# Sun-Sir/BSARec

Hardware: AMD Instinct MI355X
Metric: train sequences/sec, ML-1M L=50 d=64 2-layer (higher is better)
Workload: dtype f32

## Files before the change

bsarec_amd/_lib.py:

```python
import ctypes as C
import os

HERE = os.path.dirname(os.path.abspath(__file__))
LIB_PATH = os.environ.get("BSAREC_LIB") or os.path.join(HERE, "libbsarec_hip.so")
MAX_LAYERS = 16
ABI_VERSION = 10
TOPK_MAX = 1024
NEG_MAX = 1024
NEG_MAX_DRAWS = 1 << 20
TRAIN_NEG_MAX = 8192
TRAIN_NEG_SITE = 0x4E454753

(BUF_LAYER_OUT, BUF_LOGITS, BUF_LOSS, BUF_DSP, BUF_HMIX, BUF_PROBS, BUF_DLAYER_IN, BUF_LOSS_ROWS, BUF_CTX,
 BUF_DLOGITS, BUF_TRAIN_CAND, BUF_TRAIN_CORR, BUF_TRAIN_LOGITS, BUF_TRAIN_DLOGITS) = range(14)
K_NONE, K_FFN1, K_FFN2, K_QKV, K_LOGITS, K_DU, K_DW1, K_FUSED_FWD, K_FUSED_BWD = range(9)

LAYER_FIELDS = ["sqrt_beta", "filter_ln_w", "filter_ln_b", "query_w", "query_b", "key_w", "key_b", "value_w", "value_b",
                "dense_w", "dense_b", "attn_ln_w", "attn_ln_b", "ffn1_w", "ffn1_b", "ffn2_w", "ffn2_b", "ffn_ln_w",
                "ffn_ln_b"]
LAYER_KEYS = {
    "sqrt_beta": "layer.filter_layer.sqrt_beta",
    "filter_ln_w": "layer.filter_layer.LayerNorm.weight", "filter_ln_b": "layer.filter_layer.LayerNorm.bias",
    "query_w": "layer.attention_layer.query.weight", "query_b": "layer.attention_layer.query.bias",
    "key_w": "layer.attention_layer.key.weight", "key_b": "layer.attention_layer.key.bias",
    "value_w": "layer.attention_layer.value.weight", "value_b": "layer.attention_layer.value.bias",
    "dense_w": "layer.attention_layer.dense.weight", "dense_b": "layer.attention_layer.dense.bias",
    "attn_ln_w": "layer.attention_layer.LayerNorm.weight", "attn_ln_b": "layer.attention_layer.LayerNorm.bias",
    "ffn1_w": "feed_forward.dense_1.weight", "ffn1_b": "feed_forward.dense_1.bias",
    "ffn2_w": "feed_forward.dense_2.weight", "ffn2_b": "feed_forward.dense_2.bias",
    "ffn_ln_w": "feed_forward.LayerNorm.weight", "ffn_ln_b": "feed_forward.LayerNorm.bias",
}
OPTIONAL_LAYER_KEYS = {"filter_cw": "layer.filter_layer.complex_weight"}
TOP_KEYS = {"item_emb": "item_embeddings.weight", "pos_emb": "position_embeddings.weight",
            "ln_w": "LayerNorm.weight", "ln_b": "LayerNorm.bias"}


class Config(C.Structure):
    _fields_ = [("batch", C.c_int), ("seq_len", C.c_int), ("hidden", C.c_int), ("heads", C.c_int), ("layers", C.c_int),
                ("item_size", C.c_int), ("cutoff_bins", C.c_int), ("alpha", C.c_float), ("ln_eps", C.c_float),
                ("p_hidden", C.c_float), ("p_attn", C.c_float), ("filter_kind", C.c_int),
                ("hidden_act", C.c_int), ("storage", C.c_int), ("no_fused", C.c_int), ("no_prune_top", C.c_int),
                ("dw_tiled", C.c_int), ("splits", C.c_int), ("top_slabs", C.c_int), ("separate_embed", C.c_int),
                ("separate_top", C.c_int), ("chain_kernels", C.c_int), ("x3_products", C.c_int),
                ("train_negatives", C.c_int), ("train_sampler", C.c_int), ("train_no_logq", C.c_int),
                ("train_lazy_adam", C.c_int)]


TRAIN_FIELDS = ("train_negatives", "train_sampler", "train_no_logq")
TRAIN_SAMPLERS = {"uniform": 0, "popularity": 1}


OPTION_FIELDS = ("storage", "no_fused", "no_prune_top", "dw_tiled", "splits", "top_slabs", "separate_embed", "separate_top", "chain_kernels", "x3_products")
HIDDEN_ACTS = {"gelu": 0, "relu": 1, "swish": 2, "tanh": 3, "sigmoid": 4}

_defaults = {k: 0 for k in OPTION_FIELDS}


def _env_defaults():
    e = os.environ
    d = {}
    if e.get("BSAREC_DW") == "tiled":
        d["dw_tiled"] = 1
    if e.get("BSAREC_PRUNE_TOP") == "0":
        d["no_prune_top"] = 1
    if e.get("BSAREC_EMBED_IN_BLOCK") == "0":
        d["separate_embed"] = 1
    if e.get("BSAREC_TOP_TAIL") == "0":
        d["separate_top"] = 1
    if e.get("BSAREC_FUSED") == "0":
        d["no_fused"] = 1
    if e.get("BSAREC_BLOCK_KERNELS") == "chain":
        d["chain_kernels"] = 1
    if e.get("BSAREC_PRODUCTS") == "bf16x3":
        d["x3_products"] = 1
    for env, key, hi in (("BSAREC_TOP_SLABS", "top_slabs", 16), ("BSAREC_SPLITS", "splits", 1024)):
        if e.get(env, "").isdigit() and 1 <= int(e[env]) <= hi:
            d[key] = int(e[env])
    if e.get("BSAREC_STORAGE") == "bf16":
        d["storage"] = 1
    return d


def set_default_options(**kw):
    old = {}
    for k, v in kw.items():
        if k not in _defaults:
            raise KeyError(k)
        old[k] = _defaults[k]
        _defaults[k] = int(v)
    return old


def default_options():
    d = dict(_defaults)
    d.update(_env_defaults())
    return d


class Layer(C.Structure):
    _fields_ = [(f, C.c_void_p) for f in LAYER_FIELDS] + [("filter_cw", C.c_void_p)]


class Tensors(C.Structure):
    _fields_ = [("item_emb", C.c_void_p), ("pos_emb", C.c_void_p), ("ln_w", C.c_void_p), ("ln_b", C.c_void_p),
                ("layer", Layer * MAX_LAYERS)]


class Adam(C.Structure):
    _fields_ = [("params", C.c_void_p), ("grads", C.c_void_p), ("exp_avg", C.c_void_p), ("exp_avg_sq", C.c_void_p),
                ("n", C.c_long), ("lr", C.c_float), ("beta1", C.c_float), ("beta2", C.c_float), ("eps", C.c_float),
                ("weight_decay", C.c_float), ("grad_scale", C.c_float), ("shadow_bf16", C.c_void_p), ("shadow_from", C.c_long),
                ("grads2", C.c_void_p), ("grads2_n", C.c_long), ("n_grad_srcs", C.c_int), ("grad_srcs", C.c_void_p * 8)]


class Comm(C.Structure):
    _fields_ = [("rank", C.c_int), ("world", C.c_int), ("flags", C.c_void_p * 8), ("epoch", C.c_void_p),
                ("error", C.c_void_p), ("timeout_ms", C.c_int)]


HOOK = C.CFUNCTYPE(None, C.c_void_p, C.c_void_p)


EXPORTS = {
    "bsarec_abi_version": (C.c_int, []),
    "bsarec_workspace_bytes": (C.c_size_t, [C.POINTER(Config)]),
    "bsarec_plan_create": (C.c_int, [C.POINTER(C.c_void_p), C.POINTER(Config), C.POINTER(Tensors), C.POINTER(Tensors),
                                     C.POINTER(Tensors), C.c_void_p, C.c_size_t, C.c_void_p, C.c_void_p, C.c_void_p]),
    "bsarec_shadow_refresh": (C.c_int, [C.c_void_p, C.c_void_p]),
    "bsarec_plan_set_dense_grad_hook": (C.c_int, [C.c_void_p, HOOK, C.c_void_p, C.c_void_p]),
    "bsarec_plan_set_train_sampler": (C.c_int, [C.c_void_p, C.c_void_p]),
    "bsarec_buffer_is_bf16": (C.c_int, [C.c_void_p, C.c_int, C.c_int]),
    "bsarec_plan_is_fused": (C.c_int, [C.c_void_p]),
    "bsarec_config_is_fused": (C.c_int, [C.c_void_p]),
    "bsarec_plan_destroy": (None, [C.c_void_p]),
    "bsarec_buffer_offset": (C.c_long, [C.c_void_p, C.c_int, C.c_int]),
    "bsarec_step_begin": (C.c_int, [C.c_void_p, C.c_void_p]),
    "bsarec_forward": (C.c_int, [C.c_void_p, C.c_void_p, C.c_int, C.c_void_p]),
    "bsarec_forward_last": (C.c_int, [C.c_void_p, C.c_void_p, C.c_int, C.c_void_p]),
    "bsarec_loss": (C.c_int, [C.c_void_p, C.c_void_p, C.c_void_p]),
    "bsarec_loss_bce": (C.c_int, [C.c_void_p, C.c_void_p, C.c_void_p, C.c_void_p]),
    "bsarec_loss_logsig": (C.c_int, [C.c_void_p, C.c_void_p, C.c_void_p, C.c_void_p]),
    "bsarec_logits": (C.c_int, [C.c_void_p, C.c_void_p]),
    "bsarec_backward": (C.c_int, [C.c_void_p, C.c_void_p]),
    "bsarec_backward_seq": (C.c_int, [C.c_void_p, C.c_void_p, C.c_void_p]),
    "bsarec_backward_seq_multi": (C.c_int, [C.c_void_p, C.c_void_p, C.c_void_p]),
    "bsarec_adam_step": (C.c_int, [C.POINTER(Adam), C.c_void_p, C.c_void_p]),
    "bsarec_train_step": (C.c_int, [C.c_void_p, C.c_void_p, C.c_void_p, C.POINTER(Adam), C.c_void_p]),
    "bsarec_gather_batch": (C.c_int, [C.c_void_p, C.c_void_p, C.c_void_p, C.c_long, C.c_void_p, C.c_int, C.c_int,
                                      C.c_void_p, C.c_void_p, C.c_void_p]),
    "bsarec_train_step_indexed": (C.c_int, [C.c_void_p] * 4 + [C.c_long] + [C.c_void_p] * 3 + [C.POINTER(Adam), C.c_void_p]),
    "bsarec_grad_step_indexed": (C.c_int, [C.c_void_p] * 4 + [C.c_long] + [C.c_void_p] * 3 + [C.c_float] * 3 + [C.c_void_p]),
    "bsarec_adam_apply": (C.c_int, [C.POINTER(Adam), C.c_void_p, C.c_void_p]),
    "bsarec_mask_seen": (C.c_int, [C.c_void_p, C.c_long, C.c_int, C.c_void_p, C.c_void_p, C.c_void_p, C.c_void_p]),
    "bsarec_topk_seen": (C.c_int, [C.c_void_p, C.c_long, C.c_int, C.c_int, C.c_void_p, C.c_void_p, C.c_void_p, C.c_int, C.c_void_p,
                                   C.c_void_p, C.c_void_p]),
    "bsarec_sampled_rank": (C.c_int, [C.c_void_p, C.c_long, C.c_void_p, C.c_int, C.c_int, C.c_int] + [C.c_void_p] * 5 +
                            [C.c_int, C.c_uint64, C.c_uint32] + [C.c_void_p] * 4),
    "bsarec_topk_full_workspace_bytes": (C.c_long, [C.c_int] * 5),
    "bsarec_topk_full": (C.c_int, [C.c_void_p, C.c_long, C.c_void_p, C.c_int, C.c_int, C.c_int] + [C.c_void_p] * 3 +
                         [C.c_int, C.c_int, C.c_void_p, C.c_long, C.c_void_p, C.c_void_p, C.c_void_p]),
    "bsarec_freq_layer_fwd": (C.c_int, [C.c_void_p] * 5 + [C.c_int] * 4 + [C.c_float, C.c_float, C.c_void_p, C.c_int,
# ... 91 lines not shown
```

bsarec_amd/csrc/bsarec_hip.hip:

```cpp
#include <cmath>
#include "../../include/bsarec_hip.h"
#include "../../include/bsarec_shard.h"
#include "epilogues.h"
#include "kernels.h"
#include "fused_layer.h"
#include "dw_direct.h"
#include "fused_top.h"
#include "fused_chain.h"
#include "comm.h"
#include "catalogue_shard.h"
#include "sampled_rank.h"
#include "full_rank.h"
#include "sampled_softmax.h"
#include "lazy_adam.h"

#include <hip/hip_runtime.h>
#include <math.h>
#include <stdio.h>
#include <stdlib.h>
#include <string.h>
#include <vector>
#include <algorithm>

#define HIPCHK(x) do { hipError_t e_ = (x); if (e_ != hipSuccess) return (int)e_; } while (0)
// ... 36 lines not shown
    float *xhat0, *rstd0;
    LayerBufs lb[BSAREC_MAX_LAYERS];
    float *logits, *dlogits, *loss_rows, *loss;
    float *dXa, *dXb, *dz, *dT, *dU, *dH, *dXacc, *dO, *dF, *dC, *dS, *dq, *dk, *dv, *dXtmp, *dlast_slab;
    float *slab_wL[BSAREC_MAX_LAYERS], *slab_bL[BSAREC_MAX_LAYERS], *part_lnL[BSAREC_MAX_LAYERS], *part_betaL[BSAREC_MAX_LAYERS];
    float *part_ln0, *part_pos, *trash;
    int pos_slices;
    ReduceJob* jobs; int jobs_per_layer;
    ReduceJob* jobs_pruned;
    bool prune_ok;
    bool pruned;
    int loss_kind;
    const float* ext_dy = nullptr;
    const float* ext_mid[BSAREC_MAX_LAYERS] = {};
    const int64_t *bce_pos, *bce_neg;
    float *part_kvb, *slab_dummy;
    float* part_cwL[BSAREC_MAX_LAYERS];
    float *top_dq, *top_dO, *top_dT, *top_dU, *top_ak, *top_rk, *top_av, *top_rv;
    int* blockmap; int red_blocks;
    long red_elems; const float *red_lo, *red_hi;
    int top_slabs; bool embed_in_block, direct_dw;
    bool scatter_in_block;
    ProfState prof;
    long long* stamps = nullptr;
    bsarec_hook_t dense_hook = nullptr; void* dense_hook_user = nullptr;
    float* lookup_grad = nullptr;
    unsigned long long* lookup_acc = nullptr;
    int* ssm_cand = nullptr; float *ssm_corr = nullptr, *ssm_logits = nullptr, *ssm_dlogits = nullptr;
    const int64_t* pop_cum = nullptr;
    const int64_t* ssm_answers = nullptr;
    int ssm_nslab = 0;
    LazyRows lazy = {};
    bool lazy_now = false;
};
struct PlanScope {
    bsarec_plan* prev;
    explicit PlanScope(bsarec_plan* p) : prev(t_plan) { t_plan = p; }
    ~PlanScope() { t_plan = prev; }
};

struct ProfScope {
    hipStream_t s; bool on; hipEvent_t stop;
    ProfScope(int kclass, hipStream_t st) : s(st), on(false) {
        ProfState* ps = t_plan ? &t_plan->prof : nullptr;
        on = ps && kclass != BSAREC_K_NONE && kclass == ps->kclass;
        if (!on) return;
        if (ps->used == ps->events.size()) {
            hipEvent_t a, b;
            (void)hipEventCreate(&a); (void)hipEventCreate(&b);
            ps->events.push_back({a, b});
        }
        (void)hipEventRecord(ps->events[ps->used].first, s);
        stop = ps->events[ps->used].second;
        ++ps->used;
    }
    ~ProfScope() { if (on) (void)hipEventRecord(stop, s); }
};

template <auto Kernel, class... A>
static int launch_lds(dim3 grid, dim3 block, size_t smem, hipStream_t s, const A&... a) {
    static size_t raised = 0;
    if (smem > 48 * 1024 && smem > raised) {
        HIPCHK(hipFuncSetAttribute(reinterpret_cast<const void*>(Kernel), hipFuncAttributeMaxDynamicSharedMemorySize, (int)smem));
        raised = smem;
    }
    if (g_dry) return 0;
// ... 41 lines not shown
    memset(&e, 0, sizeof(e));
    e.C[0] = C; e.ldc = ldc;
    return e;
}

struct Carver {
    char* base; size_t off;
    explicit Carver(char* b) : base(b), off(0) {}
    template <class T> T* take(size_t n) {
        T* p = base ? reinterpret_cast<T*>(base + off) : nullptr;
        off += rup((long)(n * sizeof(T)), 256);
        return p;
    }
};

static int check_cfg(const bsarec_config_t& c) {
    if (c.batch < 1 || c.seq_len < 1 || c.seq_len > 256) return -1;
    if (c.hidden < 4 || c.hidden > 256 || c.hidden % 4) return -2;
    if (c.heads < 1 || c.hidden % c.heads || (c.hidden / c.heads) % 4) return -3;
    if (c.layers < 1 || c.layers > BSAREC_MAX_LAYERS) return -4;
    if (c.item_size < 2) return -5;
    if (c.cutoff_bins < 1 || c.cutoff_bins > c.seq_len / 2 + 1) return -6;
    if ((long)c.cutoff_bins * c.hidden > 8192) return -7;
    if (c.p_hidden < 0.f || c.p_hidden >= 1.f || c.p_attn < 0.f || c.p_attn >= 1.f) return -8;
    if (c.filter_kind != 0 && c.filter_kind != 1) return -9;
    if (c.filter_kind == 1 && c.cutoff_bins != c.seq_len / 2 + 1) return -9;
    if (c.hidden_act < 0 || c.hidden_act > 4) return -14;
    if (c.storage < 0 || c.storage > 1) return -15;
    if (c.splits < 0 || c.splits > 1024 || c.top_slabs < 0 || c.top_slabs > 16) return -16;
    if (c.train_negatives < 0 || c.train_negatives > BSAREC_TRAIN_NEG_MAX) return -17;
    if (c.train_sampler < 0 || c.train_sampler > 1 || c.train_no_logq < 0 || c.train_no_logq > 1) return -17;
    if (c.train_negatives > 0 && c.storage != 0) return -18;
    if (c.train_lazy_adam < 0 || c.train_lazy_adam > 1 || (c.train_lazy_adam && c.train_negatives == 0)) return -19;
    return 0;
}

static bool fused_shape_ok(const bsarec_config_t& c) {
    const int dh = c.hidden / c.heads;
    if (c.no_fused || c.hidden_act != 0 || c.hidden != 64 || c.seq_len > 64 || !(dh == 16 || dh == 32 || dh == 64)) return false;
    if (c.filter_kind == 1) return c.storage == 0 && c.alpha == 1.0f && c.cutoff_bins <= 36;
    return c.cutoff_bins <= FUSED_MAX_CB;
}

#define SSM_SLAB_MAX 32
static void ssm_split(int N, int cap, int* nslab, int* chunk) {
    const int want = std::max(1, std::min(cap, N / 256));
    *chunk = (int)rup(cdiv(N, want), SSM_KS);
    *nslab = cdiv(N, *chunk);
}

static void derive(bsarec_plan& p) {
    const bsarec_config_t& c = p.cfg;
    p.fused = fused_shape_ok(c);
    p.bf = c.storage == 1 && p.fused;
    p.bf_products = c.storage == 1 && !p.fused;
    p.T = c.batch * c.seq_len;
    p.Lp = (int)rup(c.seq_len, 4);
    p.Vp = (int)rup(c.item_size, 4);
    p.dh = c.hidden / c.heads;
    p.nblk = p.fused ? c.batch : cdiv(p.T, 64);
    p.rows_pb = p.fused ? c.seq_len : 64;
    const int want_splits = c.splits > 0 ? c.splits : (p.fused ? 32 : 40);
    p.top_slabs = c.top_slabs > 0 ? c.top_slabs : 2;
    p.embed_in_block = !c.separate_embed || p.bf;
    p.direct_dw = !c.dw_tiled && (long)p.T * 4 * c.hidden * 4 < (1L << 31);
    p.scatter_in_block = p.fused && p.direct_dw && !c.separate_embed;
    long ch = rup(cdiv(p.T, want_splits), p.bf ? 2 * GEMM_BK : GEMM_BK);
// ... 69 lines not shown
}

extern "C" int bsarec_abi_version(void) { return BSAREC_ABI_VERSION; }

extern "C" size_t bsarec_workspace_bytes(const bsarec_config_t* cfg) {
    if (!cfg || check_cfg(*cfg) != 0) return 0;
    bsarec_plan p;
    p.cfg = *cfg;
    derive(p);
    size_t total = 0;
    carve(p, nullptr, &total);
    return total;
}

struct SlabMap { long wq, wk, wv, wo, w1, w2, wtot, bq, bk, bv, bo, b1, b2, btot; };
static SlabMap slab_map(long d) {
    SlabMap m;
    m.wq = 0; m.wk = d * d; m.wv = 2 * d * d; m.wo = 3 * d * d; m.w1 = 4 * d * d; m.w2 = 8 * d * d; m.wtot = 12 * d * d;
    m.bq = 0; m.bk = d; m.bv = 2 * d; m.bo = 3 * d; m.b1 = 4 * d; m.b2 = 8 * d; m.btot = 9 * d;
    return m;
}

static float* slab_w_ptr(const bsarec_plan& p, int l, long tensor_off) { return p.slab_wL[l] + tensor_off * p.nsplit; }
static float* slab_b_ptr(const bsarec_plan& p, int l, long tensor_off) { return p.slab_bL[l] + tensor_off * p.nsplit; }

enum LnPart { LN_FF_G, LN_FF_B, LN_A_G, LN_A_B, LN_F_G, LN_F_B };
enum Ln0Part { LN_E_G, LN_E_B };
static float* ln_part(const bsarec_plan& p, int l, LnPart k) { return p.part_lnL[l] + (long)k * p.nblk * p.cfg.hidden; }
static float* ln0_part(const bsarec_plan& p, Ln0Part k) { return p.part_ln0 + (long)k * p.nblk * p.cfg.hidden; }

static const float* h_last(const bsarec_plan& p) { return p.X[p.cfg.layers] + (long)(p.cfg.seq_len - 1) * p.cfg.hidden; }
static long h_last_stride(const bsarec_plan& p) { return (long)p.cfg.seq_len * p.cfg.hidden; }

extern "C" int bsarec_plan_create(bsarec_plan_t** out, const bsarec_config_t* cfg, const bsarec_tensors_t* params,
                                  const bsarec_tensors_t* grads, const bsarec_tensors_t* shadow, void* workspace,
                                  size_t workspace_bytes, void* state, const float* twiddle, void* stream) {
    if (!out || !cfg || !params || !workspace || !state || !twiddle) return -10;
    RET(check_cfg(*cfg));
    if (cfg->storage == 1 && fused_shape_ok(*cfg) && !shadow) return -15;
    if (((uintptr_t)workspace & 255) != 0) return -11;
    bsarec_plan* p = new bsarec_plan();
    p->cfg = *cfg;
    p->P = *params;
    if (grads) p->G = *grads; else memset(&p->G, 0, sizeof(p->G));
    if (shadow) p->S = *shadow; else memset(&p->S, 0, sizeof(p->S));
    p->ws = (char*)workspace; p->ws_bytes = workspace_bytes;
    p->state = (uint64_t*)state; p->twiddle = twiddle; p->train = false;
    derive(*p);
    size_t total = 0;
    carve(*p, p->ws, &total);
    if (total > workspace_bytes) { delete p; return -12; }
    if (hipMemset(p->lookup_acc, 0, (size_t)cfg->item_size * cfg->hidden * sizeof(unsigned long long)) != hipSuccess) {
        delete p; return -12;
    }
    if (cfg->train_lazy_adam && (hipMemset(p->lazy.mark, 0, (size_t)cfg->item_size * sizeof(int)) != hipSuccess ||
                                 hipMemset(p->lazy.count, 0, sizeof(int)) != hipSuccess)) {
        delete p; return -12;
    }

    const long d = cfg->hidden;
    const SlabMap sm = slab_map(d);
    std::vector<ReduceJob> jobs;
    auto add = [&](const float* src, float* dst, int nsplit, long len) {
        ReduceJob j; j.src = src; j.dst = dst; j.nsplit = nsplit; j.len = (int)len; j.stride = len; j.scale = 1.f; j.pad = 0;
        jobs.push_back(j);
    };
    const int ns = p->nsplit, nb = p->nblk;
    for (int l = 0; l < cfg->layers; ++l) {
        const bsarec_layer_t& g = p->G.layer[l];
        add(p->part_betaL[l], g.sqrt_beta, cfg->batch, d);
        add(ln_part(*p, l, LN_F_G), g.filter_ln_w, nb, d);
        add(ln_part(*p, l, LN_F_B), g.filter_ln_b, nb, d);
        add(slab_w_ptr(*p, l, sm.wq), g.query_w, ns, d * d); add(slab_b_ptr(*p, l, sm.bq), g.query_b, ns, d);
        add(slab_w_ptr(*p, l, sm.wk), g.key_w, ns, d * d);   add(slab_b_ptr(*p, l, sm.bk), g.key_b, ns, d);
        add(slab_w_ptr(*p, l, sm.wv), g.value_w, ns, d * d); add(slab_b_ptr(*p, l, sm.bv), g.value_b, ns, d);
        add(slab_w_ptr(*p, l, sm.wo), g.dense_w, ns, d * d); add(slab_b_ptr(*p, l, sm.bo), g.dense_b, ns, d);
        add(ln_part(*p, l, LN_A_G), g.attn_ln_w, nb, d);
        add(ln_part(*p, l, LN_A_B), g.attn_ln_b, nb, d);
        add(slab_w_ptr(*p, l, sm.w1), g.ffn1_w, ns, 4 * d * d); add(slab_b_ptr(*p, l, sm.b1), g.ffn1_b, ns, 4 * d);
        add(slab_w_ptr(*p, l, sm.w2), g.ffn2_w, ns, 4 * d * d); add(slab_b_ptr(*p, l, sm.b2), g.ffn2_b, ns, d);
        add(ln_part(*p, l, LN_FF_G), g.ffn_ln_w, nb, d);
        add(ln_part(*p, l, LN_FF_B), g.ffn_ln_b, nb, d);
    }
    add(ln0_part(*p, LN_E_G), p->G.ln_w, nb, d);
    add(ln0_part(*p, LN_E_B), p->G.ln_b, nb, d);
    if (p->scatter_in_block) {
        ReduceJob j; j.src = p->dz; j.dst = p->G.pos_emb; j.nsplit = cfg->batch; j.len = (int)((long)cfg->seq_len * d);
        j.stride = (long)cfg->seq_len * d; j.scale = 1.f; j.pad = 0;
        jobs.push_back(j);
    } else add(p->part_pos, p->G.pos_emb, p->pos_slices, (long)cfg->seq_len * d);
    if (cfg->filter_kind == 1)
        for (int l = 0; l < cfg->layers; ++l)
            add(p->part_cwL[l], p->G.layer[l].filter_cw, cfg->batch, (long)cfg->cutoff_bins * d * 2);
    p->jobs_per_layer = 19;
    p->prune_ok = p->fused && cfg->layers >= 2 && !cfg->no_prune_top && cfg->filter_kind == 0;
    p->pruned = false;
    p->loss_kind = 0; p->bce_pos = nullptr; p->bce_neg = nullptr;
    std::vector<ReduceJob> jobs_pr = jobs;
    {
        const size_t base = (size_t)(cfg->layers - 1) * 19;
        ReduceJob& jk = jobs_pr[base + 6]; jk.src = p->part_kvb; jk.nsplit = cfg->batch; jk.stride = d;
        ReduceJob& jv = jobs_pr[base + 8]; jv.src = p->part_kvb + (long)cfg->batch * d; jv.nsplit = cfg->batch; jv.stride = d;
        for (int j : {3, 4, 5, 7, 9, 10, 13, 14, 15, 16})
            jobs_pr[base + j].nsplit = std::min(p->top_slabs, ns);
    }
    std::vector<int> bmap;
    for (size_t j = 0; j < jobs.size(); ++j)
        for (int ch = 0; ch < cdiv(jobs[j].len, 64); ++ch) bmap.push_back((int)(j << 16) | ch);
    p->red_blocks = (int)bmap.size();
    p->red_elems = 0; p->red_lo = nullptr; p->red_hi = nullptr;
    for (const ReduceJob& j : jobs) {
        p->red_elems += j.len;
        if (!p->red_lo || j.dst < p->red_lo) p->red_lo = j.dst;
// ... 58 lines not shown
}

extern "C" int bsarec_plan_set_train_sampler(bsarec_plan_t* p, const int64_t* pop_cum) {
    if (!p) return -10;
    if (p->cfg.train_negatives == 0 || p->cfg.train_sampler != 1) return -22;
    p->pop_cum = pop_cum;
    return 0;
}

static int sampled_refusal(const bsarec_plan& p) {
    if (p.cfg.train_negatives == 0) return 0;
    if (p.dense_hook || p.lookup_grad) return -22;
    if (p.cfg.train_sampler == 1 && !p.pop_cum && !g_dry) return -23;
    return 0;
}

static int head_nsplit(const bsarec_plan& p) { return p.loss_kind == 1 ? 1 : (p.loss_kind == 2 ? p.ssm_nslab : p.vsplit); }

extern "C" int bsarec_plan_is_fused(const bsarec_plan_t* p) { return p && p->fused ? 1 : 0; }
extern "C" int bsarec_config_is_fused(const bsarec_config_t* cfg) {
    if (!cfg) return -10;
    RET(check_cfg(*cfg));
    return fused_shape_ok(*cfg) ? 1 : 0;
}

extern "C" int bsarec_buffer_is_bf16(const bsarec_plan_t* p, int buffer, int layer) {
    if (!p || !p->bf) return 0;
    switch (buffer) {
        case BSAREC_BUF_LAYER_OUT: return layer < p->cfg.layers ? 1 : 0;
        case BSAREC_BUF_HMIX: case BSAREC_BUF_PROBS: case BSAREC_BUF_CTX: return 1;
        case BSAREC_BUF_DLAYER_IN: return 1;
        default: return 0;
    }
}

extern "C" int bsarec_shadow_refresh(bsarec_plan_t* p, void* stream) {
    if (!p) return -10;
    if (!p->bf) return 0;
    const long d = p->cfg.hidden;
    for (int l = 0; l < p->cfg.layers; ++l) {
        const bsarec_layer_t& w = p->P.layer[l];
        const bsarec_layer_t& sh = p->S.layer[l];
        CastJobs6 J;
        const float* src[6] = {w.query_w, w.key_w, w.value_w, w.dense_w, w.ffn1_w, w.ffn2_w};
        float* dst[6] = {sh.query_w, sh.key_w, sh.value_w, sh.dense_w, sh.ffn1_w, sh.ffn2_w};
        for (int i = 0; i < 6; ++i) { J.src[i] = src[i]; J.dst[i] = (unsigned short*)dst[i]; J.n4[i] = (i < 4 ? d * d : 4 * d * d) / 4; }
        hipLaunchKernelGGL(cast_bf16_kernel, dim3(cdiv(4 * d * d / 4, ROW_THREADS), 6), dim3(ROW_THREADS), 0, (hipStream_t)stream, J);
        HIPCHK(hipGetLastError());
    }
    return 0;
}

static uint32_t drop_thresh(float p) {
    double t = (double)p * 4294967296.0;
    if (t <= 0) return 0;
    if (t >= 4294967295.0) return 0xFFFFFFFFu;
    return (uint32_t)t;
}
static DropP make_drop(const bsarec_plan& p, float prob, int site, bool train) {
    DropP d;
    d.thresh = train ? drop_thresh(prob) : 0;
    d.scale = (train && prob > 0.f) ? (float)(1.0 / (1.0 - (double)prob)) : 1.0f;
    d.rng = p.state; d.site = (uint32_t)site;
    return d;
}
static int lpr_for(int d) { return d <= 64 ? 16 : (d <= 128 ? 32 : 64); }
// ... 63 lines not shown
    F.xhat_f = b.xhat_f; F.rstd_f = b.rstd_f; F.q = b.q; F.k = b.k; F.v = b.v; F.probs = b.probs;
    F.xhat_a = b.xhat_a; F.rstd_a = b.rstd_a; F.xhat_ff = b.xhat_ff; F.rstd_ff = b.rstd_ff;
    F.L = c.seq_len; F.Lp = p.Lp; F.cb = c.cutoff_bins; F.heads = c.heads;
    F.alpha = c.alpha; F.oma = (float)(1.0 - (double)c.alpha);
    F.drop_f = make_drop(p, c.p_hidden, 1 + 4 * l, tr); F.drop_p = make_drop(p, c.p_attn, 2 + 4 * l, tr);
    F.drop_o = make_drop(p, c.p_hidden, 3 + 4 * l, tr); F.drop_ff = make_drop(p, c.p_hidden, 4 + 4 * l, tr);
    F.stamps = p.stamps ? p.stamps + 32 * (2 * l + (FWD ? 0 : 1)) : nullptr;
    if constexpr (FWD) {
        F.Xout = p.X[l + 1];
        F.f_b = w.filter_ln_b; F.bq = w.query_b; F.bk = w.key_b; F.bv = w.value_b; F.bo = w.dense_b; F.a_b = w.attn_ln_b;
        F.b1 = w.ffn1_b; F.b2 = w.ffn2_b; F.ff_b = w.ffn_ln_b;
        F.ids32 = p.ids32; F.ctx = b.ctx; F.hmix = b.hmix; F.u = b.u;
        F.eps = c.ln_eps;
    }
}

template <class BlockP>
static void fill_block_partials(const bsarec_plan& p, int l, BlockP& F) {
    F.pg_ff = ln_part(p, l, LN_FF_G); F.pb_ff = ln_part(p, l, LN_FF_B); F.pg_a = ln_part(p, l, LN_A_G);
    F.pb_a = ln_part(p, l, LN_A_B); F.pg_f = ln_part(p, l, LN_F_G); F.pb_f = ln_part(p, l, LN_F_B);
    F.pbeta = p.part_betaL[l];
}

static void fill_top_fwd(bsarec_plan& p, int l, bool tr, TopFwdP& F) {
    fill_block<true>(p, l, tr, p.P.layer[l], F);
    F.low = p.lb[l].dsp;
    F.wk_sh = p.S.layer[l].key_w; F.wv_sh = p.S.layer[l].value_w;
}

static int launch_fused_fwd(bsarec_plan& p, int l, bool tr, hipStream_t s, const int64_t* ids = nullptr, const GatherP* gp = nullptr,
                            bool top_tail = false ) {
    const bsarec_config_t& c = p.cfg;
    FusedFwdP F;
    fill_block<true>(p, l, tr, p.bf ? p.S.layer[l] : p.P.layer[l], F);
    F.xout_f32 = (l == c.layers - 1);
    F.gp = p.lb[l].gp;
    F.dsp = nullptr;
    if (l == 0 && gp) {
        F.e_E = p.P.item_emb; F.e_pos = p.P.pos_emb; F.e_g = p.P.ln_w; F.e_b = p.P.ln_b; F.e_ids = ids; F.e_gp = *gp;
        F.e_drop = make_drop(p, c.p_hidden, 0, tr); F.e_V = c.item_size;
        F.e_X0 = p.X[0]; F.e_xhat = p.xhat0; F.e_rstd = p.rstd0; F.e_ids32 = p.ids32;
    }
    F.trash = p.trash;
    TopFwdP TF;
    if (top_tail) fill_top_fwd(p, l + 1, tr, TF);
    const dim3 grid(c.batch), block(512);
    ProfScope prof(BSAREC_K_FUSED_FWD, s);
    if (c.filter_kind == 1) {
        F.filter_cw = p.P.layer[l].filter_cw;
        return launch_lds<fused_layer_fwd_kernel<32, false, NoTail, false, true>>(grid, block, fused_fwd_smem_bytes(), s, F, NoTail());
    }
    int rc = 0;
    if (!p.bf && c.chain_kernels && !c.x3_products) {
        const size_t csm = fused_chain_fwd_smem_bytes(top_tail);
        DISPATCH_DH(p.dh, rc = top_tail ? launch_lds<fused_chain_fwd_kernel<DH, TopFwdP>>(grid, block, csm, s, F, TF)
                                        : launch_lds<fused_chain_fwd_kernel<DH, NoTail>>(grid, block, csm, s, F, NoTail()));
        return rc;
    }
    const size_t smem = fused_fwd_smem_bytes();
    DISPATCH_BLOCK(p, rc = top_tail ? launch_lds<fused_layer_fwd_kernel<DH, BF, TopFwdP, X3>>(grid, block, smem, s, F, TF)
                                    : launch_lds<fused_layer_fwd_kernel<DH, BF, NoTail, X3>>(grid, block, smem, s, F, NoTail()));
    return rc;
}

static int launch_fused_bwd(bsarec_plan& p, int l, bool tr, const float* dY, float* dXout, hipStream_t s, bool top,
                            const TopBwdP* head = nullptr ) {
    const bsarec_config_t& c = p.cfg;
    FusedBwdP F;
    fill_block<false>(p, l, tr, p.bf ? p.S.layer[l] : p.P.layer[l], F);
    fill_block_partials(p, l, F);
    F.dY = dY; F.dX = dXout;
    F.u = p.lb[l].gp;
    if (top) { F.dh_slabs = p.dlast_slab; F.dh_nsplit = head_nsplit(p); F.dh_stride = (long)c.batch * c.hidden; }
    if (l == 0) {
        F.e_dz = p.dz; F.e_xhat = p.xhat0; F.e_rstd = p.rstd0; F.e_g = p.P.ln_w;
        F.e_pg = ln0_part(p, LN_E_G); F.e_pb = ln0_part(p, LN_E_B); F.e_drop = make_drop(p, c.p_hidden, 0, tr);
        F.e_dx_extra = p.ext_dy ? p.ext_mid[0] : nullptr;
    }
    F.dT = p.dT; F.dU = p.dU; F.dO = p.dO; F.dq = p.dq; F.dk = p.dk; F.dv = p.dv;
    F.trash = p.trash;
    const dim3 grid(c.batch), block(512);
    const size_t smem = fused_bwd_smem_bytes();
    ProfScope prof(BSAREC_K_FUSED_BWD, s);
    if (c.filter_kind == 1) {
        F.filter_cw = p.P.layer[l].filter_cw; F.pcw = p.part_cwL[l];
        return launch_lds<fused_layer_bwd_kernel<32, false, NoTail, false, true>>(grid, block, smem, s, F, NoTail());
    }
    int rc = 0;
    DISPATCH_BLOCK(p, rc = head ? launch_lds<fused_layer_bwd_kernel<DH, BF, TopBwdP, X3>>(grid, block, smem, s, F, *head)
                                : launch_lds<fused_layer_bwd_kernel<DH, BF, NoTail, X3>>(grid, block, smem, s, F, NoTail()));
    return rc;
}

static int launch_top_fwd(bsarec_plan& p, int l, bool tr, hipStream_t s) {
    TopFwdP F;
    fill_top_fwd(p, l, tr, F);
    int rc = 0;
    DISPATCH_BLOCK(p, rc = launch_lds<top_fwd_kernel<DH, BF>>(dim3(p.cfg.batch), dim3(256), top_fwd_smem_bytes(), s, F));
    return rc;
}

static void fill_top_bwd(bsarec_plan& p, int l, bool tr, float* dXout, TopBwdP& F) {
    const bsarec_config_t& c = p.cfg;
    fill_block<false>(p, l, tr, p.P.layer[l], F);
    fill_block_partials(p, l, F);
    F.dX = dXout;
    F.u = p.lb[l].u; F.low = p.lb[l].dsp;
    F.dh_slabs = p.dlast_slab; F.dh_nsplit = head_nsplit(p); F.dh_stride = (long)c.batch * c.hidden;
    F.dT = p.top_dT; F.dU = p.top_dU; F.dO = p.top_dO; F.dq = p.top_dq;
    F.ak = p.top_ak; F.rk = p.top_rk; F.av = p.top_av; F.rv = p.top_rv;
    F.pbk = p.part_kvb; F.pbv = p.part_kvb + (long)c.batch * c.hidden;
}

static int launch_top_bwd(bsarec_plan& p, int l, bool tr, float* dXout, hipStream_t s) {
    TopBwdP F;
    fill_top_bwd(p, l, tr, dXout, F);
    int rc = 0;
    DISPATCH_BLOCK(p, rc = launch_lds<top_bwd_kernel<DH, BF>>(dim3(p.cfg.batch), dim3(256), top_bwd_smem_bytes(), s, F));
    return rc;
}

// ... 534 lines not shown
}

static int launch_dw_grouped(const bsarec_plan& p, const GroupedTN& G, hipStream_t s) {
    ProfScope prof(BSAREC_K_DW1, s);
    const dim3 grid(G.tile0[6], p.nsplit), block(GEMM_THREADS);
    if (!p.bf_products)
        return launch_lds<gemm_grouped_tn_kernel<false, 64>>(grid, block, GemmSmem<64, 64, true, true, false>::BYTES, s, G);
    if (dw_tile(p) == 128)
        return launch_lds<gemm_grouped_tn_kernel<true, 128>>(grid, block, GemmSmem<128, 128, true, true, true>::BYTES, s, G);
    return launch_lds<gemm_grouped_tn_kernel<true, 64>>(grid, block, GemmSmem<64, 64, true, true, true>::BYTES, s, G);
}

static int embed_bwd(bsarec_plan& p, const float* dY, hipStream_t s) {
    const bsarec_config_t& c = p.cfg;
    const int T = p.T, d = c.hidden, L = c.seq_len, B = c.batch;
    if (!p.fused) {
        LnBranch a; memset(&a, 0, sizeof(a));
        a.xhat = p.xhat0; a.rstd = p.rstd0; a.gamma = p.P.ln_w; a.in_scale = 1.f;
        a.drop = make_drop(p, c.p_hidden, 0, p.train); a.dT = nullptr;
        a.pgamma = ln0_part(p, LN_E_G); a.pbeta = ln0_part(p, LN_E_B);
        DISPATCH_LPR(d, LAUNCH((ln_bwd_kernel<LPR, 2>), dim3(p.nblk), dim3(ROW_THREADS), 0, s, dY, a, a, p.dz, T, d, p.rows_pb));
        HIPCHK(hipGetLastError());
    }
    if (!p.scatter_in_block)
    DISPATCH_LPR(d, {
        constexpr int CHUNK = SCATTER_FLOATS / (LPR * 4);
        const int sb = cdiv(T, CHUNK);
        RET(launch_lds<embed_bwd_kernel<LPR>>(dim3(sb + L * p.pos_slices), dim3(ROW_THREADS), SCATTER_FLOATS * 8 + 2 * CHUNK * 4, s,
                                              p.dz, p.ids32, B, L, d, p.lookup_acc, p.part_pos, sb));
    });
    return 0;
}

static int final_reduce(bsarec_plan& p, const TickP& tick, const bsarec_adam_t* fuse_adam, hipStream_t s) {
    const bsarec_config_t& c = p.cfg;
    LookupAcc la;
    memset(&la, 0, sizeof(la));
    la.acc = p.lookup_acc; la.dst = p.lookup_grad ? p.lookup_grad : p.G.item_emb; la.n4 = (long)c.item_size * c.hidden / 4;
    la.nblocks = (int)std::min<long>(cdiv(la.n4, ROW_THREADS), 1024);
    la.dense_zero = (!p.ext_dy && p.loss_kind == 2) ? 1 : 0;
    const bool lazy = p.lazy_now && !p.ext_dy && p.loss_kind == 2;
    if (lazy) {
        la.lazy = p.lazy;
        la.nblocks = (int)std::min<long>(cdiv((long)p.lazy.cap * p.lazy.d4, ROW_THREADS), 1024);
    }
    const ReduceJob* jobs = p.pruned ? p.jobs_pruned : p.jobs;
    if (fuse_adam) {
        const bsarec_adam_t& a = *fuse_adam;
        AdamFuseP A;
        memset(&A, 0, sizeof(A));
        A.w = a.params; A.g = const_cast<float*>(a.grads); A.m = a.exp_avg; A.v = a.exp_avg_sq;
        A.b1 = a.beta1; A.b2 = a.beta2; A.eps = a.eps; A.wd = a.weight_decay;
        A.shadow = (unsigned short*)a.shadow_bf16; A.shadow_from = a.shadow_bf16 ? a.shadow_from : a.n;
        A.item_off = p.G.item_emb - a.grads; A.item_n4 = la.n4; A.lookup_acc = la.acc;
        A.dense_zero = la.dense_zero;
        if (lazy) A.lazy = p.lazy;
        int ab = lazy ? la.nblocks : cdiv(A.item_n4, ROW_THREADS);
        if (ab > 1024) ab = 1024;
        LAUNCH(reduce_adam_kernel, dim3(p.red_blocks + ab), dim3(ROW_THREADS), 0, s, jobs, p.blockmap, p.red_blocks,
               (const uint64_t*)p.state, A);
    } else
        LAUNCH(multi_reduce_flat_kernel, dim3(p.red_blocks + la.nblocks + (tick.state ? 1 : 0)), dim3(ROW_THREADS), 0, s, jobs,
               p.blockmap, p.red_blocks, tick, la);
    return (int)hipGetLastError();
}

static int backward_impl(bsarec_plan_t* p, void* stream, const TickP& tick, const bsarec_adam_t* fuse_adam) {
    if (!p) return -10;
    if (!p->G.item_emb) return -13;
    if (fuse_adam && p->lookup_grad) return -21;
    PlanScope scope(p);
    hipStream_t s = (hipStream_t)stream;
    const bsarec_config_t& c = p->cfg;
    const int T = p->T, d = c.hidden, L = c.seq_len, B = c.batch, N = c.layers;
    const bool tr = p->train;

    RET(head_bwd(*p, s));
    if (p->dense_hook && !g_dry && !p->ext_dy) p->dense_hook(p->dense_hook_user, stream);
    float* dY = (N & 1) ? p->dXb : p->dXa;
    RET(top_grad(*p, dY, s));

    DwPending pend;
    memset(&pend, 0, sizeof(pend));
    for (int l = N - 1; l >= 0; --l) {
        float* dXout = (dY == p->dXa) ? p->dXb : p->dXa;
        const bool top_pruned = p->fused && p->pruned && l == N - 1;
        if (top_pruned) {
            if (N >= 2 && !c.separate_top && p->direct_dw) { fill_top_bwd(*p, l, tr, dXout, pend.top_head); pend.have_head = true; }
// ... 25 lines not shown
}

static TickP make_tick(void* state, int adam, float lr, float b1, float b2, const float* loss_rows, int B, float* loss_out,
                       void* cursor, int advance, int bump_step) {
    TickP t;
    memset(&t, 0, sizeof(t));
    t.state = (uint64_t*)state; t.adam = adam; t.lr = lr; t.b1 = b1; t.b2 = b2;
    t.loss_rows = loss_rows; t.B = B; t.loss_out = loss_out;
    t.cursor = (long long*)cursor; t.advance = advance; t.bump_step = bump_step;
    return t;
}

static int adam_check(const bsarec_adam_t* a) {
    if (!a || !a->params || !a->grads || !a->exp_avg || !a->exp_avg_sq || a->n <= 0 || (a->n & 3)) return -10;
    if (a->shadow_bf16 && (a->shadow_from < 0 || (a->shadow_from & 3))) return -10;
    if (a->grads2 && (a->grads2_n < 0 || a->grads2_n > a->n || (a->grads2_n & 3))) return -10;
    if (a->n_grad_srcs < 0 || a->n_grad_srcs > 8) return -10;
    for (int r = 0; r < a->n_grad_srcs; ++r) if (!a->grad_srcs[r]) return -10;
    return 0;
}

static int adam_launch(const bsarec_adam_t& a, void* state, hipStream_t s) {
    const long n4 = a.n / 4;
    int blocks = cdiv(n4, ROW_THREADS);
    if (blocks > 2048) blocks = 2048;
    GradSrcs S;
    memset(&S, 0, sizeof(S));
    S.nsrc = a.n_grad_srcs;
    for (int r = 0; r < a.n_grad_srcs; ++r) S.src[r] = a.grad_srcs[r];
    S.g2 = a.grads2; S.n2_4 = a.grads2 ? a.grads2_n / 4 : 0;
    LAUNCH(adam_kernel, dim3(blocks), dim3(ROW_THREADS), 0, s, a.params, a.grads, a.exp_avg, a.exp_avg_sq, n4,
           (const uint64_t*)state, a.beta1, a.beta2, a.eps, a.weight_decay, a.grad_scale, (unsigned short*)a.shadow_bf16,
           a.shadow_bf16 ? a.shadow_from / 4 : n4, S);
    return (int)hipGetLastError();
}

extern "C" int bsarec_adam_step(const bsarec_adam_t* a, void* state, void* stream) {
    RET(adam_check(a));
    if (!state) return -10;
    hipStream_t s = (hipStream_t)stream;
    LAUNCH(adam_tick_kernel, dim3(1), dim3(ROW_THREADS), 0, s, make_tick(state, 1, a->lr, a->beta1, a->beta2, nullptr, 0, nullptr, nullptr, 0, 0));
    HIPCHK(hipGetLastError());
    return adam_launch(*a, state, s);
}

extern "C" int bsarec_adam_apply(const bsarec_adam_t* a, void* state, void* stream) {
    RET(adam_check(a));
    if (!state) return -10;
    return adam_launch(*a, state, (hipStream_t)stream);
}

static int lazy_check(const bsarec_plan& p, const bsarec_adam_t& a) {
    if (!p.cfg.train_lazy_adam) return 0;
    if (a.grads2 || a.n_grad_srcs > 0 || a.shadow_bf16) return -24;
    const long item = (long)p.cfg.item_size * p.cfg.hidden;
    if (!p.G.item_emb || p.G.item_emb < a.grads) return -24;
    const long off = p.G.item_emb - a.grads;
    if (off + item > a.n || (off & 3)) return -24;
    return 0;
}

static int lazy_adam_launch(const bsarec_plan& p, const bsarec_adam_t& a, hipStream_t s) {
    LazyAdamP A;
    memset(&A, 0, sizeof(A));
    A.w = a.params; A.g = a.grads; A.m = a.exp_avg; A.v = a.exp_avg_sq;
    A.n = a.n; A.item_off = p.G.item_emb - a.grads; A.item_n = (long)p.cfg.item_size * p.cfg.hidden;
    A.b1 = a.beta1; A.b2 = a.beta2; A.eps = a.eps; A.wd = a.weight_decay; A.gscale = a.grad_scale;
// ... 5 lines not shown
}

struct LazyStep {
    bsarec_plan* p;
    explicit LazyStep(bsarec_plan* q) : p(q) { p->lazy_now = p->cfg.train_lazy_adam != 0; }
    ~LazyStep() { p->lazy_now = false; }
};

extern "C" int bsarec_gather_batch(const int64_t* table, const int64_t* answers_table, const int64_t* perm, long n_samples,
                                   const void* cursor, int B, int L, int64_t* ids_out, int64_t* answers_out, void* stream) {
    if (!table || !answers_table || !perm || !cursor || !ids_out || !answers_out || B < 1 || L < 1) return -10;
    LAUNCH(gather_batch_kernel, dim3(cdiv((long)B * L, ROW_THREADS)), dim3(ROW_THREADS), 0, (hipStream_t)stream, table,
           answers_table, perm, n_samples, (const long long*)cursor, B, L, ids_out, answers_out);
    return (int)hipGetLastError();
}

extern "C" int bsarec_train_step_indexed(bsarec_plan_t* p, const int64_t* table, const int64_t* answers_table,
                                         const int64_t* perm, long n_samples, void* cursor, int64_t* ids_buf,
                                         int64_t* answers_buf, const bsarec_adam_t* a, void* stream) {
    if (!p) return -10;
    RET(adam_check(a));
    RET(sampled_refusal(*p));
    RET(lazy_check(*p, *a));
    hipStream_t s = (hipStream_t)stream;
    if (!table || !answers_table || !perm || !cursor || !ids_buf || !answers_buf) return -10;
    LazyStep lazy(p);
    GatherP gp{table, answers_table, perm, n_samples, (const long long*)cursor, ids_buf, answers_buf};
    RET(forward_impl(p, ids_buf, 1, stream, gp, true));
    RET(loss_impl(p, answers_buf, stream, false));
    const TickP tk = make_tick(p->state, 1, a->lr, a->beta1, a->beta2, p->loss_rows, p->cfg.batch, p->loss, cursor, p->cfg.batch, 1);
    if (can_fuse_adam(*p, *a) && !p->cfg.separate_embed)
        return backward_impl(p, stream, tk, a);
    RET(backward_impl(p, stream, tk));
    return p->lazy_now ? lazy_adam_launch(*p, *a, s) : adam_launch(*a, p->state, s);
}

extern "C" int bsarec_grad_step_indexed(bsarec_plan_t* p, const int64_t* table, const int64_t* answers_table,
                                        const int64_t* perm, long n_samples, void* cursor, int64_t* ids_buf,
                                        int64_t* answers_buf, float lr, float b1, float b2, void* stream) {
    if (!p || !table || !answers_table || !perm || !cursor || !ids_buf || !answers_buf) return -10;
    RET(sampled_refusal(*p));
    if (p->cfg.train_lazy_adam) return -22;
    GatherP gp{table, answers_table, perm, n_samples, (const long long*)cursor, ids_buf, answers_buf};
    RET(forward_impl(p, ids_buf, 1, stream, gp, true));
    RET(bsarec_loss(p, answers_buf, stream));
    return backward_impl(p, stream, make_tick(p->state, lr > 0.f ? 1 : 0, lr, b1, b2, nullptr, 0, nullptr, cursor, p->cfg.batch, 1));
}

extern "C" int bsarec_train_step(bsarec_plan_t* p, const int64_t* ids, const int64_t* answers, const bsarec_adam_t* a,
                                 void* stream) {
    if (!p) return -10;
    RET(adam_check(a));
    RET(sampled_refusal(*p));
    RET(lazy_check(*p, *a));
    if (p->cfg.train_lazy_adam) {
        LazyStep lazy(p);
        RET(bsarec_step_begin(p, stream));
        RET(bsarec_forward_last(p, ids, 1, stream));
        RET(bsarec_loss(p, answers, stream));
        TickP tk = make_tick(p->state, 1, a->lr, a->beta1, a->beta2, nullptr, 0, nullptr, nullptr, 0, 0);
        RET(backward_impl(p, stream, tk));
        return lazy_adam_launch(*p, *a, (hipStream_t)stream);
    }
    RET(bsarec_step_begin(p, stream));
    RET(bsarec_forward_last(p, ids, 1, stream));
    RET(bsarec_loss(p, answers, stream));
    RET(bsarec_backward(p, stream));
    return bsarec_adam_step(a, p->state, stream);
}

extern "C" int bsarec_mask_seen(float* scores, long ld, int B, const int64_t* users, const int64_t* indptr,
                                const int64_t* indices, void* stream) {
    if (!scores || !users || !indptr || !indices || B < 1 || ld < 1) return -10;
    hipLaunchKernelGGL(mask_seen_kernel, dim3(B), dim3(ROW_THREADS), 0, (hipStream_t)stream, scores, ld, users, indptr, indices);
    return (int)hipGetLastError();
}

extern "C" int bsarec_topk_seen(float* scores, long ld, int B, int V, const int64_t* users, const int64_t* indptr,
                                const int64_t* indices, int k, int64_t* out_idx, float* out_val, void* stream) {
    static_assert(BSAREC_TOPK_MAX == TOPK_MAX && ROW_THREADS == 256, "topk_seen_kernel: one thread per digit bin");
    if (!scores || !out_idx || B < 1 || V < 1 || ld < V || k < 1 || k > BSAREC_TOPK_MAX || k > V) return -10;
    if (indptr && (!users || !indices)) return -10;
    hipLaunchKernelGGL(topk_seen_kernel, dim3(B), dim3(ROW_THREADS), 0, (hipStream_t)stream, scores, ld, V, users, indptr, indices, k,
                       out_idx, out_val);
    return (int)hipGetLastError();
}

extern "C" int bsarec_sampled_rank(const float* h, long ldh, const float* item_emb, int B, int V, int d, const int64_t* users,
                                   const int64_t* answers, const int64_t* indptr, const int64_t* indices, const int64_t* pop_cum,
                                   int n_neg, uint64_t seed, uint32_t tag, int32_t* rank_out, int64_t* cand_out, float* score_out,
                                   void* stream) {
    static_assert(BSAREC_NEG_MAX == NEG_MAX && BSAREC_NEG_MAX_DRAWS == NEG_MAX_DRAWS, "sampled_rank_kernel: the header's limits");
    if (!h || !item_emb || !users || !answers || !rank_out || (indptr && !indices)) return -10;
    if (B < 1 || V < 2 || d < 4 || d > 256 || d % 4 != 0 || ldh < d || n_neg < 1 || n_neg > BSAREC_NEG_MAX) return -10;
    if ((uintptr_t)item_emb % 16 != 0) return -10;
    hipLaunchKernelGGL(sampled_rank_kernel, dim3(B), dim3(ROW_THREADS), 0, (hipStream_t)stream, h, ldh, item_emb, V, d, users, answers,
                       indptr, indices, pop_cum, n_neg, (uint32_t)seed, (uint32_t)(seed >> 32), tag, rank_out, cand_out, score_out);
    return (int)hipGetLastError();
}

struct FrShape { long s, stride, cap; };
// ... 364 lines not shown
```

bsarec_amd/csrc/fused_layer.h:

```cpp
#pragma once
#include "common.h"
#include "kernels.h"
#include <type_traits>

#define FS 68
#define FU 260
#define FUSED_MAX_CB 8

struct FusedFwdP {
    const float* X; float* Xout;
    const float *sqrt_beta, *f_g, *f_b, *wq, *bq, *wk, *bk, *wv, *bv, *wo, *bo, *a_g, *a_b, *w1, *b1, *w2, *b2, *ff_g, *ff_b;
    const float* tw; const int* ids32;
    float *xhat_f, *rstd_f, *q, *k, *v, *probs, *ctx, *xhat_a, *rstd_a, *hmix, *u, *xhat_ff, *rstd_ff, *dsp;
    float* gp;
    int L, Lp, cb, heads;
    float alpha, oma, eps;
    DropP drop_f, drop_p, drop_o, drop_ff;
    float* trash;
    long long* stamps;
    const float *e_E, *e_pos, *e_g, *e_b; const int64_t* e_ids; GatherP e_gp; DropP e_drop; int e_V;
    float *e_X0, *e_xhat, *e_rstd; int* e_ids32;
    int xout_f32;
    const float* filter_cw;
};


template <class T> struct GlobalPtr { static __device__ __forceinline__ T fix(T v) { return v; } };
template <class U> struct GlobalPtr<U*> {
    static __device__ __forceinline__ U* fix(U* v) {
        return (U*)(__attribute__((address_space(1))) U*)v;
    }
};
template <class T>
__device__ __forceinline__ T kernarg_field(unsigned byte_off) {
    typedef __attribute__((address_space(4))) const char* kptr_t;
// ... 121 lines not shown
        const float c = tab[2 * (k * 64 + t)] * w, sn = tab[2 * (k * 64 + t) + 1] * w;
        low += ld4(spec + (k * 2 + 0) * 64 + lc) * c - ld4(spec + (k * 2 + 1) * 64 + lc) * sn;
    }
    return low * (1.0f / (float)L);
}

template <int MM, int K> struct WFrag;
template <int K> struct WFrag<0, K> { f32x4 w[K / 8]; };
template <int K> struct WFrag<1, K> { u32x4 w[K / 16]; };
template <int K> struct WFrag<2, K> { f32x4 w[K / 8]; };

struct Split3 { u32x4 h, m, l; };
__device__ __forceinline__ f32x4 bf_lo4(const u32x4& p, int half) {
    return half == 0 ? f32x4{bf_lo(p.x), bf_hi(p.x), bf_lo(p.y), bf_hi(p.y)} : f32x4{bf_lo(p.z), bf_hi(p.z), bf_lo(p.w), bf_hi(p.w)};
}
__device__ __forceinline__ Split3 split3(f32x4 a0, f32x4 a1) {
    Split3 r;
    r.h = pk8(a0, a1);
    a0 = a0 - bf_lo4(r.h, 0); a1 = a1 - bf_lo4(r.h, 1);
    r.m = pk8(a0, a1);
    a0 = a0 - bf_lo4(r.m, 0); a1 = a1 - bf_lo4(r.m, 1);
    r.l = pk8(a0, a1);
    return r;
}
__device__ __forceinline__ f32x16 mfma_x3(const Split3& a, const Split3& b, f32x16 acc) {
    acc = mfma_bf16(a.l, b.h, acc);
    acc = mfma_bf16(a.h, b.l, acc);
    acc = mfma_bf16(a.m, b.m, acc);
    acc = mfma_bf16(a.m, b.h, acc);
    acc = mfma_bf16(a.h, b.m, acc);
    return mfma_bf16(a.h, b.h, acc);
}

template <int MM, int K>
__device__ __forceinline__ void load_w(const float* __restrict__ base, long e, WFrag<MM, K>& f) {
    if constexpr (MM == 1) {
#pragma unroll
        for (int s = 0; s < K / 16; ++s) f.w[s] = *reinterpret_cast<const AS_GLOBAL u32x4*>((const AS_GLOBAL char*)base + 2 * (e + 16 * s));
    } else if constexpr (MM == 2) {
#pragma unroll
        for (int s = 0; s < K / 16; ++s) { f.w[2 * s] = gld4(base + e + 16 * s); f.w[2 * s + 1] = gld4(base + e + 16 * s + 4); }
    } else {
#pragma unroll
        for (int kb = 0; kb < K / 8; ++kb) f.w[kb] = gld4(base + e + 8 * kb);
    }
}
template <int MM, int K, int LDW>
__device__ __forceinline__ void load_wT(const float* __restrict__ base, long e, WFrag<MM, K>& f) {
    if constexpr (MM == 1) {
        const AS_GLOBAL unsigned short* g = reinterpret_cast<const AS_GLOBAL unsigned short*>((const AS_GLOBAL char*)base + 2 * e);
#pragma unroll
        for (int s = 0; s < K / 16; ++s) {
            unsigned h[8];
#pragma unroll
            for (int j = 0; j < 8; ++j) h[j] = g[(16 * s + j) * LDW];
            f.w[s] = u32x4{h[0] | (h[1] << 16), h[2] | (h[3] << 16), h[4] | (h[5] << 16), h[6] | (h[7] << 16)};
        }
    } else if constexpr (MM == 2) {
        const float* gw = base + e;
#pragma unroll
        for (int s = 0; s < K / 16; ++s) {
            f.w[2 * s] = f32x4{gld(gw + (16 * s + 0) * LDW), gld(gw + (16 * s + 1) * LDW), gld(gw + (16 * s + 2) * LDW), gld(gw + (16 * s + 3) * LDW)};
            f.w[2 * s + 1] = f32x4{gld(gw + (16 * s + 4) * LDW), gld(gw + (16 * s + 5) * LDW), gld(gw + (16 * s + 6) * LDW), gld(gw + (16 * s + 7) * LDW)};
        }
    } else {
        const float* gw = base + e;
#pragma unroll
        for (int kb = 0; kb < K / 8; ++kb) {
            f.w[kb].x = gld(gw + (8 * kb + 0) * LDW); f.w[kb].y = gld(gw + (8 * kb + 1) * LDW);
            f.w[kb].z = gld(gw + (8 * kb + 2) * LDW); f.w[kb].w = gld(gw + (8 * kb + 3) * LDW);
        }
    }
}
template <int MM, int K>
__device__ __forceinline__ void mma_w(const float* __restrict__ sa, const WFrag<MM, K>& f, f32x16& acc) {
    if constexpr (MM == 1) {
#pragma unroll
        for (int s = 0; s < K / 16; ++s) acc = mfma_bf16(pk8(ld4(sa + 16 * s), ld4(sa + 16 * s + 4)), f.w[s], acc);
    } else if constexpr (MM == 2) {
#pragma unroll
        for (int s = 0; s < K / 16; ++s)
            acc = mfma_x3(split3(ld4(sa + 16 * s), ld4(sa + 16 * s + 4)), split3(f.w[2 * s], f.w[2 * s + 1]), acc);
// ... 50 lines not shown
        const bool ok = r < L;
        const long e = (tok0 + r) * 64 + lc;
        f32x4 v = {0, 0, 0, 0};
        if (ok) v = (ld4(tileA + r * FS + lc) + ld4(tileB + r * FS + lc) + P.bi) * P.dm[i] + ld4(resid + r * FS + lc);
        const float mean = group_sum<16>(v.x + v.y + v.z + v.w) * (1.0f / 64.0f);
        f32x4 dl = {0, 0, 0, 0};
        if (ok) dl = v - mean;
        const float var = group_sum<16>(dl.x * dl.x + dl.y * dl.y + dl.z * dl.z + dl.w * dl.w) * (1.0f / 64.0f);
        const float rs = 1.0f / sqrtf(var + eps);
        f32x4 y = {0, 0, 0, 0};
        if (ok) {
            const f32x4 xh = dl * rs;
            y = P.g * xh + P.be;
            if (MIX) y = alpha * ld4(dsp + r * FS + lc) + oma * y;
            ast4<BF>(xhatG, e, xh);
            if (BF && out_f32) gst4(outG + e, y); else ast4<BF>(outG, e, y);
            if (lc == 0) gst(rstdG + tok0 + r, rs);
        }
        if (BF && round_outL) {
            const unsigned a = pk_bf16(y.x, y.y), c = pk_bf16(y.z, y.w);
            y = f32x4{bf_lo(a), bf_hi(a), bf_lo(c), bf_hi(c)};
        }
        if (outL) st4(outL + r * FS + lc, y);
    }
}

struct NoTail {};
template <bool BF> struct TopFwdRegs;
template <bool BF, unsigned KOFF, bool KV> __device__ __forceinline__ void top_fwd_prefetch(TopFwdRegs<BF>& R);
template <int DH, bool BF, unsigned KOFF, bool HELPED>
__device__ __forceinline__ void top_fwd_rest(const TopFwdRegs<BF>& R, const DropSeed& dseed, float* sX, float* sK, float* sV,
                                             float* sPart, float* sTab, float* sSpec, float* sVec, const int* sIds);
template <bool BF> struct TopFwdHelpRegs;
template <bool BF, unsigned KOFF> __device__ __forceinline__ void top_fwd_help_prefetch(TopFwdHelpRegs<BF>& H);
template <int DH, bool BF, unsigned KOFF>
__device__ __forceinline__ void top_fwd_help(const TopFwdHelpRegs<BF>& H, const float* sX, float* sK, float* sV, float* sVec);
template <class T> struct IsTail { static constexpr bool value = true; };
template <> struct IsTail<NoTail> { static constexpr bool value = false; };
constexpr int TOP_BWD_BARRIERS = 11;
struct TopBwdRegs {
    float sl[32];
    float xh_ff, g_ff, rs_ff, xa, xf, g_a, g_f, rs_a, rs_f, bt, low_l, x_l, q_l;
    f32x4 tq[16];
    float p_pre;
};
struct TopBwdHelpRegs { f32x4 w2c[16], w1c[16], u4; };
template <bool BF, unsigned KOFF> __device__ __forceinline__ void top_bwd_prefetch(TopBwdRegs& R);
template <bool BF, unsigned KOFF> __device__ __forceinline__ void top_bwd_prefetch_tile(TopBwdRegs& R);
template <bool BF, unsigned KOFF> __device__ __forceinline__ void top_bwd_help_prefetch(TopBwdHelpRegs& H);
template <int DH, bool BF, unsigned KOFF, bool HELPED>
__device__ __forceinline__ void top_bwd_body(const TopBwdRegs& R, const DropSeed& dseed, float* sX, float* sK, float* sV, const float* sTab,
                                             float* sVec, float* sDX);
template <bool BF, unsigned KOFF> __device__ __forceinline__ void top_bwd_help_a(const TopBwdHelpRegs& H, float* sVec);
template <int DH, bool BF, unsigned KOFF> __device__ __forceinline__ void top_bwd_help_b(const float* sX, float* sVec, const float* gu, f32x4 (&uw)[16]);


template <int DH, bool BF, class TAILP, bool X3 = false, bool FM = false>
__global__ void __launch_bounds__(512) __attribute__((amdgpu_waves_per_eu(2, 2)))
fused_layer_fwd_kernel(const FusedFwdP P_unused, const TAILP T_unused) {
#define PTYPE FusedFwdP
    static_assert(!(BF && X3), "x3 products work on fp32 tensors");
    constexpr int MM = X3 ? 2 : (BF ? 1 : 0);
    static_assert(!FM || (!BF && !X3 && !IsTail<TAILP>::value), "the FMLPRec block runs in fp32, without a top-block tail");
    constexpr int MAXCB = FM ? 36 : FUSED_MAX_CB;
    constexpr bool TAIL = IsTail<TAILP>::value;
    constexpr unsigned KOFF = (unsigned)((sizeof(FusedFwdP) + 7) & ~(size_t)7);
    const auto R0_L = KARG(FusedFwdP, L);
    const auto R0_Lp = KARG(FusedFwdP, Lp);
    const auto R0_cb = KARG(FusedFwdP, cb);
    const auto R0_heads = KARG(FusedFwdP, heads);
    extern __shared__ __attribute__((aligned(16))) float sm[];
    constexpr int TS = 64 * FS;
    float* sX = sm;
    float* sD = sm + TS;
    float* sH = sm + 2 * TS;
    float* sE = sm + 3 * TS;
    float* sR = sm + 4 * TS;
    float* sQ = sR;
    float* sK = sR + TS;
    float* sVt = sR + 2 * TS;
    float* sC = sR + 3 * TS;
    float* sU = sR;
    float* sTab = sR + 4 * TS;
    float* sSpec = sTab + FUSED_MAX_CB * 128;
    float* sRed = sSpec + FUSED_MAX_CB * 128;
    int* sIds = reinterpret_cast<int*>(sRed + 512);
    if constexpr (FM) { sTab = sR; sSpec = sR + 2 * TS; }

    const int tid = threadIdx.x, lane = tid & 63, wave = tid >> 6;
    const int l31 = lane & 31, half = lane >> 5;
    const int grp = wave >> 2, wm = (wave >> 1) & 1, wn = wave & 1;
    const int L = R0_L, Lp = R0_Lp, heads = R0_heads, cb = R0_cb;
    const int b = blockIdx.x;
    const long tok0 = (long)b * L;
    const int col = wn * 32 + l31;
    constexpr int KHM = MM ? 8 : 4;
    const int KH = KHM * half;
    const long wrow = (long)col * 64 + KH;
    const int arow = (wm * 32 + l31) * FS + KH;
    float* const trash = KARG(FusedFwdP, trash) + 4 * lane;

    STAMP(0);
    const KernargTouch ktouch = kernarg_touch<IsTail<TAILP>::value ? KOFF + (unsigned)sizeof(TAILP) : (unsigned)sizeof(FusedFwdP)>();
    const DropSeed dseed = drop_seed(KARG(FusedFwdP, drop_f));
    kernarg_touch_done(ktouch);
    const auto R1_X = KARG(FusedFwdP, X);
    const auto R1_ids32 = KARG(FusedFwdP, ids32);
    const auto R1_tw = KARG(FusedFwdP, tw);
    const auto R1_wq = KARG(FusedFwdP, wq);
    WFrag<MM, 64> wA, wB;
    float qkv_bias[3] = {0.f, 0.f, 0.f};
    if (!FM && grp == 1) {
        load_w<MM, 64>(R1_wq, wrow, wA);
        qkv_bias[0] = gld(KARG(FusedFwdP, bq) + col); qkv_bias[1] = gld(KARG(FusedFwdP, bk) + col);
        qkv_bias[2] = gld(KARG(FusedFwdP, bv) + col);
    }
    const float* const eE = KARG(FusedFwdP, e_E);
    if (eE) {
        const GatherP gp = KARG(FusedFwdP, e_gp);
        const int64_t* const eids = KARG(FusedFwdP, e_ids);
        const float* const epos = KARG(FusedFwdP, e_pos);
        const int V = KARG(FusedFwdP, e_V);
        const float eeps = KARG(FusedFwdP, eps);
        const float* const e_g = KARG(FusedFwdP, e_g); const float* const e_b = KARG(FusedFwdP, e_b);
        int* const e_ids32 = KARG(FusedFwdP, e_ids32); const DropP e_drop = KARG(FusedFwdP, e_drop);
        float* const e_xhat = KARG(FusedFwdP, e_xhat); float* const e_X0 = KARG(FusedFwdP, e_X0); float* const e_rstd = KARG(FusedFwdP, e_rstd);
        long src = 0;
        if (gp.table) {
            src = *(const AS_GLOBAL long long*)gp.cursor + b;
            src = src < gp.n ? (long)*(const AS_GLOBAL int64_t*)(gp.perm + src) : 0;
            if (tid == 0) *(AS_GLOBAL int64_t*)(gp.ans_out + b) = *(const AS_GLOBAL int64_t*)(gp.ans_table + src);
        }
        const f32x4 eg = gld4(e_g + ((tid & 15) << 2)), eb = gld4(e_b + ((tid & 15) << 2));
#pragma unroll
        for (int p = 0; p < 2; ++p) {
            const int idx = tid + p * 512, r = idx >> 4, c4 = (idx & 15) << 2;
            const bool ok = r < L;
            const long e = (tok0 + r) * 64 + c4;
            f32x4 v = {0, 0, 0, 0};
            int id = 0;
            if (ok) {
                int64_t id64;
                if (gp.table) {
                    id64 = *(const AS_GLOBAL int64_t*)(gp.table + src * L + r);
                    if (c4 == 0) *(AS_GLOBAL int64_t*)(gp.ids_out + tok0 + r) = id64;
                } else id64 = *(const AS_GLOBAL int64_t*)(eids + tok0 + r);
// ... 26 lines not shown
        st4(sX + r * FS + c4, v);
    }
    if (tid < 64) sIds[tid] = tid < L ? gldi(R1_ids32 + (tok0 + tid)) : 0;
    }
    build_twiddle_table(R1_tw, L, cb, sTab);
    lds_barrier();

    STAMP(1);
    const auto R2_bk = KARG(FusedFwdP, bk);
    const auto R2_bq = KARG(FusedFwdP, bq);
    const auto R2_bv = KARG(FusedFwdP, bv);
    const auto R2_drop_f = KARG(FusedFwdP, drop_f);
    const auto R2_dsp = KARG(FusedFwdP, dsp);
    const auto R2_eps = KARG(FusedFwdP, eps);
    const auto R2_f_b = KARG(FusedFwdP, f_b);
    const auto R2_f_g = KARG(FusedFwdP, f_g);
    const auto R2_k = KARG(FusedFwdP, k);
    const auto R2_q = KARG(FusedFwdP, q);
    const auto R2_rstd_f = KARG(FusedFwdP, rstd_f);
    const auto R2_sqrt_beta = KARG(FusedFwdP, sqrt_beta);
    const auto R2_v = KARG(FusedFwdP, v);
    const auto R2_wk = KARG(FusedFwdP, wk);
    const auto R2_wo = KARG(FusedFwdP, wo);
    const auto R2_wv = KARG(FusedFwdP, wv);
    const auto R2_xhat_f = KARG(FusedFwdP, xhat_f);
    {
        float* part = sH;
        const int lr = (tid & 255) >> 4, lc = (tid & 15) << 2;
        auto qkv = [&](auto whichc) {
            constexpr int which = decltype(whichc)::value;
            f32x16 acc;
#pragma unroll
            for (int r = 0; r < 16; ++r) acc[r] = 0.f;
            if (which == 0) { load_w<MM, 64>(R2_wk, wrow, wB); mma_w<MM, 64>(sX + arow, wA, acc); }
            else if (which == 1) { load_w<MM, 64>(R2_wv, wrow, wA); mma_w<MM, 64>(sX + arow, wB, acc); }
            else mma_w<MM, 64>(sX + arow, wA, acc);
            const float bias = qkv_bias[which];
#pragma unroll
            for (int r = 0; r < 16; ++r) {
                const int row = wm * 32 + rho(r) + 4 * half;
                const float val = acc[r] + bias;
                if (which == 0) sQ[row * FS + col] = val;
                else if (which == 1) sK[row * FS + col] = val;
                else sVt[col * FS + row] = val;
            }
        };
#pragma unroll
        for (int ch = 0; ch < MAXCB / 4; ++ch) {
            const int k0 = 4 * ch;
            if (k0 >= cb) break;
            if (grp == 0) {
                f32x4 re[4], im[4];
#pragma unroll
                for (int j = 0; j < 4; ++j) { re[j] = f32x4{0, 0, 0, 0}; im[j] = f32x4{0, 0, 0, 0}; }
#pragma unroll
                for (int r0 = 0; r0 < 64; r0 += 16) {
                    const int t = r0 + lr;
                    if (t < L) {
                        const f32x4 x = ld4(sX + t * FS + lc);
#pragma unroll
                        for (int j = 0; j < 4; ++j)
                            if (k0 + j < cb) {
                                const float c = sTab[2 * ((k0 + j) * 64 + t)], sn = sTab[2 * ((k0 + j) * 64 + t) + 1];
                                re[j] += x * c; im[j] -= x * sn;
                            }
                    }
                }
#pragma unroll
// ... 34 lines not shown
            if constexpr (FM) b2 = f32x4{0, 0, 0, 0};
            float* const R2_hmix = KARG(FusedFwdP, hmix);
            const f32x4 g = gld4(R2_f_g + lc), be = gld4(R2_f_b + lc);
            const int rbeg = grp == 0 ? 0 : 48, rend = grp == 0 ? 48 : 64;
            for (int r0 = rbeg; r0 < rend; r0 += 16) {
                const int t = r0 + lr;
                const bool ok = t < L;
                const long e = (tok0 + t) * 64 + lc;
                f32x4 v = {0, 0, 0, 0};
                if (ok) {
                    const f32x4 xv = ld4(sX + t * FS + lc);
                    const f32x4 low = lowpass_tab(sSpec, t, lc, L, cb, sTab);
                    v = (low + b2 * (xv - low)) * drop_mult4(R2_drop_f, dseed, (uint64_t)e >> 2) + xv;
                }
                const float mean = group_sum<16>(v.x + v.y + v.z + v.w) * (1.0f / 64.0f);
                f32x4 dl = {0, 0, 0, 0};
                if (ok) dl = v - mean;
                const float var = group_sum<16>(dl.x * dl.x + dl.y * dl.y + dl.z * dl.z + dl.w * dl.w) * (1.0f / 64.0f);
                const float rs = 1.0f / sqrtf(var + R2_eps);
                f32x4 y = {0, 0, 0, 0};
                if (ok) {
                    const f32x4 xh = dl * rs;
                    y = g * xh + be;
                    ast4<BF>(R2_xhat_f, e, xh);
                    if (R2_dsp) gst4(R2_dsp + e, y);
                    if constexpr (FM) gst4(R2_hmix + e, y);
                    if (lc == 0) gst(R2_rstd_f + (tok0 + t), rs);
                }
                st4((FM ? sH : sD) + t * FS + lc, y);
            }
        }
    }
    WFrag<MM, 32> wO;
    if constexpr (!FM) load_w<MM, 32>(R2_wo, wrow + 32 * grp, wO);
    lds_barrier();
    if constexpr (!FM) {
    {
        const int lr = tid >> 4, lc = (tid & 15) << 2;
#pragma unroll
        for (int r0 = 0; r0 < 64; r0 += 32) {
            const int r = r0 + lr;
            if (r < L) {
                const long e = (tok0 + r) * 64 + lc;
                ast4<BF>(R2_q, e, ld4(sQ + r * FS + lc));
                ast4<BF>(R2_k, e, ld4(sK + r * FS + lc));
                ast4<BF>(R2_v, e, f32x4{sVt[lc * FS + r], sVt[(lc + 1) * FS + r], sVt[(lc + 2) * FS + r], sVt[(lc + 3) * FS + r]});
            }
        }
    }

    STAMP(3);
    const auto R3_ctx = KARG(FusedFwdP, ctx);
    const auto R3_drop_p = KARG(FusedFwdP, drop_p);
    const auto R3_probs = KARG(FusedFwdP, probs);
    {
        const int nt = (L + 31) >> 5;
        const float sqrt_dh = sqrtf((float)DH);
        constexpr int NCT = (DH + 31) / 32;
        const int ncombo = heads * nt;
        const int pair = wave >> 1, kt = wave & 1;
        for (int c0 = 0; c0 < ncombo; c0 += 4) {
            const int combo = c0 + pair;
            const bool act = combo < ncombo && kt < nt;
            const int head = act ? combo / nt : 0, qt = act ? combo % nt : 0;
            const int query = 32 * qt + l31;
            f32x16 st;
#pragma unroll
// ... 87 lines not shown
            lds_barrier();
        }
        {
            const int lr = tid >> 4, lc = (tid & 15) << 2;
#pragma unroll
            for (int r0 = 0; r0 < 64; r0 += 32) {
                const int r = r0 + lr;
                f32x4 v = {0, 0, 0, 0};
                if (r < 32 * nt) { v = ld4(sC + r * FS + lc); if (nt == 2) v += ld4(sE + r * FS + lc); }
                st4(sC + r * FS + lc, v);
                if (r < L) ast4<BF>(R3_ctx, (tok0 + r) * 64 + lc, v);
            }
        }
    }
    lds_barrier();
    }

    STAMP(4);
    const auto R4_a_b = KARG(FusedFwdP, a_b);
    const auto R4_a_g = KARG(FusedFwdP, a_g);
    const auto R4_alpha = KARG(FusedFwdP, alpha);
    const auto R4_bo = KARG(FusedFwdP, bo);
    const auto R4_drop_o = KARG(FusedFwdP, drop_o);
    const auto R4_eps = KARG(FusedFwdP, eps);
    const auto R4_hmix = KARG(FusedFwdP, hmix);
    const auto R4_oma = KARG(FusedFwdP, oma);
    const auto R4_rstd_a = KARG(FusedFwdP, rstd_a);
    const auto R4_w1 = KARG(FusedFwdP, w1);
    const auto R4_xhat_a = KARG(FusedFwdP, xhat_a);
    float ffn_bias[2];
    LnPre lnA;
    if constexpr (!FM) lnA = ln_pre(R4_bo, R4_a_g, R4_a_b, R4_drop_o, dseed, tok0);
    {
        load_w<MM, 64>(R4_w1, (long)(128 * grp + col) * 64 + KH, wA);
        ffn_bias[0] = gld(KARG(FusedFwdP, b1) + 128 * grp + col); ffn_bias[1] = gld(KARG(FusedFwdP, b1) + 128 * grp + 64 + col);
        if constexpr (!FM) {
        f32x16 acc;
#pragma unroll
        for (int r = 0; r < 16; ++r) acc[r] = 0.f;
        mma_w<MM, 32>(sC + arow + 32 * grp, wO, acc);
        float* part = grp == 0 ? sQ : sK;
#pragma unroll
        for (int r = 0; r < 16; ++r) part[(wm * 32 + rho(r) + 4 * half) * FS + col] = acc[r];
        }
    }
    if constexpr (!FM) {
    lds_barrier();
    ln_rows_64<true, BF>(lnA, sQ, sK, sX, R4_eps, sD, R4_alpha, R4_oma, tok0, L, sH, R4_hmix, R4_xhat_a, R4_rstd_a);
    lds_barrier();
    }

    STAMP(5);
    const auto R5_b1 = KARG(FusedFwdP, b1);
    const auto R5_u = KARG(FusedFwdP, u);
    const auto R5_w1 = KARG(FusedFwdP, w1);
    const auto R5_w2 = KARG(FusedFwdP, w2);
    {
        const float* sa = sH + arow;
#pragma unroll
        for (int i = 0; i < 2; ++i) {
            const int c256 = (2 * grp + i) * 64 + col;
            WFrag<MM, 64>& wcur = i ? wB : wA;
            WFrag<MM, 64>& wnxt = i ? wA : wB;
            if (i == 0) load_w<MM, 64>(R5_w1, (long)(c256 + 64) * 64 + KH, wnxt);
            else load_w<MM, 64>(R5_w2, (long)col * 256 + 128 * grp + KH, wnxt);
            f32x16 acc;
#pragma unroll
            for (int r = 0; r < 16; ++r) acc[r] = 0.f;
            mma_w<MM, 64>(sa, wcur, acc);
            const float bias = ffn_bias[i];
#pragma unroll
            for (int r = 0; r < 16; ++r) {
                const int row = wm * 32 + rho(r) + 4 * half;
                sU[row * FU + c256] = acc[r] + bias;
            }
        }
    }
    lds_barrier();

    STAMP(6);
    const auto R6_w2 = KARG(FusedFwdP, w2);
    const auto R6_u = KARG(FusedFwdP, u);
    const auto R6_gp = KARG(FusedFwdP, gp);
    const auto R7_b2 = KARG(FusedFwdP, b2);
    const auto R7_drop_ff = KARG(FusedFwdP, drop_ff);
    const auto R7_ff_b = KARG(FusedFwdP, ff_b);
    const auto R7_ff_g = KARG(FusedFwdP, ff_g);
    LnPre lnF;
    {
        for (int idx = tid; idx < 64 * 64; idx += 512) {
            const int r = idx >> 6, c4 = (idx & 63) << 2;
            const f32x4 v = ld4(sU + r * FU + c4);
            float g0, g1, g2, g3, p0, p1, p2, p3;
            gelu_both(v.x, g0, p0); gelu_both(v.y, g1, p1); gelu_both(v.z, g2, p2); gelu_both(v.w, g3, p3);
            const f32x4 g = {g0, g1, g2, g3}, gp = {p0, p1, p2, p3};
            if (r < L) { ast4<BF>(R6_u, (tok0 + r) * 256 + c4, g); ast4<BF>(R6_gp, (tok0 + r) * 256 + c4, gp); }
            st4(sU + r * FU + c4, g);
        }
        lds_barrier();
        lnF = ln_pre(R7_b2, R7_ff_g, R7_ff_b, R7_drop_ff, dseed, tok0);
        f32x16 acc;
#pragma unroll
        for (int r = 0; r < 16; ++r) acc[r] = 0.f;
        const float* sa = sU + (wm * 32 + l31) * FU + 128 * grp + KH;
        load_w<MM, 64>(R6_w2, (long)col * 256 + 128 * grp + 64 + KH, wB);
        mma_w<MM, 64>(sa, wA, acc);
        mma_w<MM, 64>(sa + 64, wB, acc);
        float* part = grp == 0 ? sX : sE;
#pragma unroll
        for (int r = 0; r < 16; ++r) part[(wm * 32 + rho(r) + 4 * half) * FS + col] = acc[r];
    }
    lds_barrier();
    STAMP(7);
    TopFwdRegs<BF> TR;
    TopFwdHelpRegs<BF> TH;
    if constexpr (TAIL) { if (wave < 4) top_fwd_prefetch<BF, KOFF, false>(TR); else top_fwd_help_prefetch<BF, KOFF>(TH); }
    const auto R7_Xout = KARG(FusedFwdP, Xout);
    const auto R7_eps = KARG(FusedFwdP, eps);
    const auto R7_rstd_ff = KARG(FusedFwdP, rstd_ff);
    const auto R7_xhat_ff = KARG(FusedFwdP, xhat_ff);
    ln_rows_64<false, BF>(lnF, sX, sE, sH, R7_eps, nullptr, 0.f, 1.f, tok0, L,
                          TAIL ? sD : nullptr, R7_Xout, R7_xhat_ff, R7_rstd_ff, KARG(FusedFwdP, xout_f32) != 0, TAIL);
    STAMP(8);
    if constexpr (TAIL) {
        lds_barrier();
        if (wave < 4) top_fwd_rest<DH, BF, KOFF, true>(TR, dseed, sD, sR, sR + TS, sR + 2 * TS, sTab, sSpec, sX, sIds);
        else top_fwd_help<DH, BF, KOFF>(TH, sD, sR, sR + TS, sX);
    }
}
#undef PTYPE

static inline size_t fused_fwd_smem_bytes() {
    return (size_t)(8 * 64 * FS + 2 * FUSED_MAX_CB * 128 + 512 + 64) * 4;
}

struct FusedBwdP {
    const float* dY; float* dX; const float* X;
    const float *sqrt_beta, *f_g, *wq, *wk, *wv, *wo, *a_g, *w1, *w2, *ff_g;
    const float* tw;
    const float *xhat_f, *rstd_f, *q, *k, *v, *probs, *xhat_a, *rstd_a, *u, *xhat_ff, *rstd_ff;
    const float* dh_slabs; int dh_nsplit; long dh_stride;
    float *dT, *dU, *dO, *dq, *dk, *dv;
    float *pg_ff, *pb_ff, *pg_a, *pb_a, *pg_f, *pb_f, *pbeta;
    int L, Lp, cb, heads;
    float alpha, oma;
    DropP drop_f, drop_p, drop_o, drop_ff;
    float* trash;
    long long* stamps;
    float* e_dz; const float *e_xhat, *e_rstd, *e_g; float *e_pg, *e_pb; DropP e_drop;
// ... 13 lines not shown
        float s = 0.f;
        for (int g = 0; g < ng; ++g) s += red[g * 64 + threadIdx.x];
        if (mul) s *= gld(mul + threadIdx.x);
        gst(dst + threadIdx.x, s * scale_by);
    }
}


template <int N>
__device__ __forceinline__ void seq_partials_64(const f32x4 (&v)[N], float* const (&red)[N], float* const (&dst)[N],
                                                float scale0 = 1.f, const float* __restrict__ mul0 = nullptr) {
    const int lr = threadIdx.x >> 4, lc = (threadIdx.x & 15) << 2;
    const int ng = blockDim.x >> 4;
    lds_barrier();
#pragma unroll
    for (int i = 0; i < N; ++i) st4(red[i] + lr * 64 + lc, v[i]);
    lds_barrier();
    const int i = threadIdx.x >> 6, c = threadIdx.x & 63;
    if (i < N) {
        const float* r = red[0];
        float* d = dst[0];
#pragma unroll
        for (int k = 1; k < N; ++k) if (i == k) { r = red[k]; d = dst[k]; }
        float s0 = 0.f, s1 = 0.f, s2 = 0.f, s3 = 0.f;
        for (int g = 0; g < ng; g += 4) {
            s0 += r[g * 64 + c]; s1 += r[(g + 1) * 64 + c]; s2 += r[(g + 2) * 64 + c]; s3 += r[(g + 3) * 64 + c];
        }
        float sum = (s0 + s1) + (s2 + s3);
        if (i == 0) { if (mul0) sum *= gld(mul0 + c); sum *= scale0; }
        gst(d + c, sum);
    }
}

template <int DH, bool BF, class HEADP, bool X3 = false, bool FM = false>
__global__ void __launch_bounds__(512) __attribute__((amdgpu_waves_per_eu(2, 2)))
fused_layer_bwd_kernel(const FusedBwdP P_unused, const HEADP H_unused) {
#define PTYPE FusedBwdP
    static_assert(!(BF && X3), "x3 products work on fp32 tensors");
    constexpr int MM = X3 ? 2 : (BF ? 1 : 0);
    static_assert(!FM || (!BF && !X3 && !IsTail<HEADP>::value), "the FMLPRec block runs in fp32, without a top-block head");
    constexpr bool HEAD = IsTail<HEADP>::value;
    constexpr unsigned KOFF = (unsigned)((sizeof(FusedBwdP) + 7) & ~(size_t)7);
    const auto R0_L = KARG(FusedBwdP, L);
    const auto R0_Lp = KARG(FusedBwdP, Lp);
    const auto R0_cb = KARG(FusedBwdP, cb);
    const auto R0_heads = KARG(FusedBwdP, heads);
    extern __shared__ __attribute__((aligned(16))) float sm[];
    constexpr int TS = 64 * FS;
    float* sAcc = sm;
    float* sT = sm + TS;
    float* sQ = sm + 2 * TS;
    float* sK = sm + 3 * TS;
    float* sV = sm + 4 * TS;
    float* sS = sm + 5 * TS;
    float* sdU = sQ;
    float* sG = sm + 6 * TS;
    float* sdF = sm + 7 * TS;
    float* sPm = sm + 8 * TS;
    float* sTab = sm + 9 * TS;
    float* sRed = sTab + FUSED_MAX_CB * 128;
    const int tid = threadIdx.x, lane = tid & 63, wave = tid >> 6;
    const int l31 = lane & 31, half = lane >> 5;
    const int grp = wave >> 2, wm = (wave >> 1) & 1, wn = wave & 1;
    const int lr = tid >> 4, lc = (tid & 15) << 2;
    const int L = R0_L, Lp = R0_Lp, heads = R0_heads, cb = R0_cb;
    const int b = blockIdx.x;
    const long tok0 = (long)b * L;
    const int col = wn * 32 + l31;
    constexpr int KHM = MM ? 8 : 4;
    const int KH = KHM * half;
    const int arow = (wm * 32 + l31) * FS + KH;
// ... 13 lines not shown
    const DropSeed dseed = drop_seed(KARG(FusedBwdP, drop_f));
    kernarg_touch_done(ktouch);
    const auto R1_dT = KARG(FusedBwdP, dT);
    const auto R1_dY = KARG(FusedBwdP, dY);
    const auto R1_dh_nsplit = KARG(FusedBwdP, dh_nsplit);
    const auto R1_dh_slabs = KARG(FusedBwdP, dh_slabs);
    const auto R1_dh_stride = KARG(FusedBwdP, dh_stride);
    const auto R1_drop_ff = KARG(FusedBwdP, drop_ff);
    const auto R1_ff_g = KARG(FusedBwdP, ff_g);
    const auto R1_pb_ff = KARG(FusedBwdP, pb_ff);
    const auto R1_pg_ff = KARG(FusedBwdP, pg_ff);
    const auto R1_rstd_ff = KARG(FusedBwdP, rstd_ff);
    const auto R1_tw = KARG(FusedBwdP, tw);
    const auto R1_w2 = KARG(FusedBwdP, w2);
    const auto R1_xhat_ff = KARG(FusedBwdP, xhat_ff);
    if constexpr (!FM && !HEAD) build_twiddle_table(R1_tw, L, cb, sTab);
    if constexpr (HEAD) {
        if (wave < 4) {
            top_bwd_body<DH, BF, KOFF, true>(HR, dseed, sG, sdF, sPm, sTab, sAcc, sT);
        } else {
            top_bwd_help_a<BF, KOFF>(HH, sAcc);
            f32x4 uw[16];
            top_bwd_help_b<DH, BF, KOFF>(sG, sAcc, KARG(FusedBwdP, u), uw);
#pragma unroll
            for (int i = 0; i < 16; ++i) {
                const int idx = (tid - 256) + i * 256, r = idx >> 6, c4 = (idx & 63) << 2;
                st4(sdU + r * FU + c4, r < L ? uw[i] : f32x4{0, 0, 0, 0});
            }
        }
    }
    WFrag<MM, 64> wA, wB;
    WFrag<MM, 32> wk4;
    f32x4 e_bt, e_x[2];
    load_wT<MM, 64, 256>(R1_w2, (long)KH * 256 + 128 * grp + col, wA);
    const f32x4 g = gld4(R1_ff_g + lc);
    f32x4 dy[2], xh[2];
    float rs[2];
#pragma unroll
    for (int i = 0; i < 2; ++i) {
        const int r = 32 * i + lr;
        const long e = (tok0 + r) * 64 + lc;
        dy[i] = f32x4{0, 0, 0, 0}; xh[i] = dy[i]; rs[i] = 0.f;
        if (R1_dh_slabs) {
            if (r < L) {
                if (r == L - 1)
                    for (int sp = 0; sp < R1_dh_nsplit; ++sp) dy[i] += gld4(R1_dh_slabs + sp * R1_dh_stride + (long)b * 64 + lc);
                xh[i] = ald4<BF>(R1_xhat_ff, e); rs[i] = gld(R1_rstd_ff + tok0 + r);
            }
        } else {
            const bool ok = r < L;
            const long ec = (tok0 + min(r, L - 1)) * 64 + lc;
            f32x4 d4 = {0, 0, 0, 0};
            if constexpr (!HEAD) d4 = ald4<BF>(R1_dY, ec);
            const f32x4 x4 = ald4<BF>(R1_xhat_ff, ec);
            const float r1 = gld(R1_rstd_ff + tok0 + min(r, L - 1));
            if constexpr (HEAD) d4 = ld4(sT + r * FS + lc);
            dy[i] = ok ? d4 : f32x4{0, 0, 0, 0}; xh[i] = ok ? x4 : f32x4{0, 0, 0, 0}; rs[i] = ok ? r1 : 0.f;
        }
    }
    f32x4 uv[8];
    if constexpr (!HEAD)
    {
        const float* gu = KARG(FusedBwdP, u);
#pragma unroll
        for (int i = 0; i < 8; ++i) {
            const int idx = tid + i * 512, r = idx >> 6, c4 = (idx & 63) << 2;
            uv[i] = ald4<BF>(gu, (tok0 + min(r, L - 1)) * 256 + c4);
// ... 11 lines not shown
            const float m1 = group_sum<16>(gg.x + gg.y + gg.z + gg.w) * (1.0f / 64.0f);
            const float m2 = group_sum<16>(gg.x * xh[i].x + gg.y * xh[i].y + gg.z * xh[i].z + gg.w * xh[i].w) * (1.0f / 64.0f);
            const f32x4 dz = rs[i] * (gg - m1 - xh[i] * m2);
            sg += dy[i] * xh[i]; sb += dy[i];
            f32x4 dt = {0, 0, 0, 0};
            if (ok) { dt = dz * drop_mult4(R1_drop_ff, dseed, (uint64_t)e >> 2); ast4<BF>(R1_dT, e, dt); }
            st4(sAcc + r * FS + lc, dz);
            st4(sT + r * FS + lc, dt);
        }
        {
            const f32x4 pv[2] = {sg, sb};
            float* const pr[2] = {sPm, sPm + 2048};
            float* const pd[2] = {R1_pg_ff + (long)b * 64, R1_pb_ff + (long)b * 64};
            seq_partials_64<2>(pv, pr, pd);
        }
    }
    if constexpr (!HEAD) {
#pragma unroll
    for (int i = 0; i < 8; ++i) {
        const int idx = tid + i * 512, r = idx >> 6, c4 = (idx & 63) << 2;
        st4(sdU + r * FU + c4, r < L ? uv[i] : f32x4{0, 0, 0, 0});
    }
    }
    lds_barrier();

    STAMP(1);
    const auto R2_dU = KARG(FusedBwdP, dU);
    const auto R2_u = KARG(FusedBwdP, u);
    const auto R2_w1 = KARG(FusedBwdP, w1);
    const auto R2_w2 = KARG(FusedBwdP, w2);
    if constexpr (MM == 0) {
        const float* sa = sT + arow;
        const int c0 = (2 * grp) * 64 + col, c1 = c0 + 64;
        load_wT<MM, 64, 256>(R2_w2, (long)KH * 256 + c1, wB);
        f32x16 acc0, acc1;
#pragma unroll
        for (int r = 0; r < 16; ++r) { acc0[r] = 0.f; acc1[r] = 0.f; }
        mma_w<MM, 64>(sa, wA, acc0);
        load_wT<MM, 64, 64>(R2_w1, (long)(128 * grp + KH) * 64 + col, wA);
#pragma unroll
        for (int r = 0; r < 16; ++r) {
            const f32x4 a = ld4(sa + 8 * (r >> 1));
            const int s0 = 2 * (r & 1);
            acc1 = __builtin_amdgcn_mfma_f32_32x32x2f32(a[s0], wB.w[r >> 1][s0], acc1, 0, 0, 0);
            acc1 = __builtin_amdgcn_mfma_f32_32x32x2f32(a[s0 + 1], wB.w[r >> 1][s0 + 1], acc1, 0, 0, 0);
            const int row = wm * 32 + rho(r) + 4 * half;
            float* pu = sdU + row * FU + c0;
            *pu = row < L ? acc0[r] * *pu : 0.f;
        }
#pragma unroll
        for (int r = 0; r < 16; ++r) {
            const int row = wm * 32 + rho(r) + 4 * half;
            float* pu = sdU + row * FU + c1;
            *pu = row < L ? acc1[r] * *pu : 0.f;
        }
    } else {
        const float* sa = sT + arow;
#pragma unroll
        for (int i = 0; i < 2; ++i) {
            const int blk = 2 * grp + i, c256 = blk * 64 + col;
            WFrag<MM, 64>& wcur = i ? wB : wA;
            WFrag<MM, 64>& wnxt = i ? wA : wB;
            if (i == 0) load_wT<MM, 64, 256>(R2_w2, (long)KH * 256 + c256 + 64, wnxt);
            else load_wT<MM, 64, 64>(R2_w1, (long)(128 * grp + KH) * 64 + col, wnxt);
            f32x16 acc;
#pragma unroll
            for (int r = 0; r < 16; ++r) acc[r] = 0.f;
            mma_w<MM, 64>(sa, wcur, acc);
#pragma unroll
            for (int r = 0; r < 16; ++r) {
                const int row = wm * 32 + rho(r) + 4 * half;
                float* pu = sdU + row * FU + c256;
                *pu = row < L ? acc[r] * *pu : 0.f;
            }
        }
    }
    lds_barrier();
    for (int idx = tid; idx < 64 * 64; idx += 512) {
        const int r = idx >> 6, c4 = (idx & 63) << 2;
        if (r < L) ast4<BF>(R2_dU, (tok0 + r) * 256 + c4, ld4(sdU + r * FU + c4));
    }

    STAMP(2);
    const auto R3_w1 = KARG(FusedBwdP, w1);
    const auto R3_wo = KARG(FusedBwdP, wo);
    WFrag<MM, 32> wO;
    f32x4 pq[2], pk[2], pv[2], xa[2], xf[2];
    float ra[2], rf[2];
    {
        f32x16 acc;
#pragma unroll
        for (int r = 0; r < 16; ++r) acc[r] = 0.f;
        const float* sa = sdU + (wm * 32 + l31) * FU + 128 * grp + KH;
        load_wT<MM, 64, 64>(R3_w1, (long)(128 * grp + 64 + KH) * 64 + col, wB);
        if constexpr (!FM) load_wT<MM, 32, 64>(R3_wo, (long)(32 * grp + KH) * 64 + col, wO);
#pragma unroll
        for (int i = 0; i < 2; ++i) {
            const int r = 32 * i + lr;
            const long ec = (tok0 + min(r, L - 1)) * 64 + lc;
            if constexpr (!FM) {
            pq[i] = ald4<BF>(KARG(FusedBwdP, q), ec); pk[i] = ald4<BF>(KARG(FusedBwdP, k), ec); pv[i] = ald4<BF>(KARG(FusedBwdP, v), ec);
            xa[i] = ald4<BF>(KARG(FusedBwdP, xhat_a), ec); ra[i] = gld(KARG(FusedBwdP, rstd_a) + tok0 + min(r, L - 1));
            }
            xf[i] = ald4<BF>(KARG(FusedBwdP, xhat_f), ec);
            rf[i] = gld(KARG(FusedBwdP, rstd_f) + tok0 + min(r, L - 1));
        }
        mma_w<MM, 64>(sa, wA, acc);
        mma_w<MM, 64>(sa + 64, wB, acc);
        float* part = grp == 0 ? sG : sdF;
#pragma unroll
        for (int r = 0; r < 16; ++r) part[(wm * 32 + rho(r) + 4 * half) * FS + col] = acc[r];
    }
    lds_barrier();

    STAMP(3);
    if constexpr (FM) {
        float* const sXin = sT;  float* const sdFm = sPm;  float* const tab = sV;  float* const spec = sG;
        const DropP drop_f = KARG(FusedBwdP, drop_f);
        const f32x4 gf = gld4(KARG(FusedBwdP, f_g) + lc);
        const float* const Xg = KARG(FusedBwdP, X);
        f32x4 sgf = {0, 0, 0, 0}, sbf = sgf;
        const f32x4 z4 = {0, 0, 0, 0};
        f32x4 dzf2[2], dF2[2], x2[2];
#pragma unroll
        for (int i = 0; i < 2; ++i) {
            const int r = 32 * i + lr;
            const bool ok = r < L;
            const long e = (tok0 + r) * 64 + lc;
// ... 313 lines not shown
                            if (!cok) { w0 = 0.f; w1 = 0.f; w2 = 0.f; w3 = 0.f; }
                            acc = __builtin_amdgcn_mfma_f32_32x32x2f32(a.x, w0, acc, 0, 0, 0);
                            acc = __builtin_amdgcn_mfma_f32_32x32x2f32(a.y, w1, acc, 0, 0, 0);
                            acc = __builtin_amdgcn_mfma_f32_32x32x2f32(a.z, w2, acc, 0, 0, 0);
                            acc = __builtin_amdgcn_mfma_f32_32x32x2f32(a.w, w3, acc, 0, 0, 0);
                        }
                        }
                    }
                }
                res[ti] = acc;
            }
            lds_barrier();
#pragma unroll
            for (int ti = 0; ti < NRES; ++ti) {
                const int t = wave + 8 * ti;
                if (t < 6 * NCT) {
                    const int kind = t / (2 * NCT), rt = (t / NCT) & 1, ct = t % NCT;
                    const int c = 32 * ct + l31;
                    if (c < DH) {
                        float* sdst = kind == 0 ? sQ : kind == 1 ? sK : sV;
#pragma unroll
                        for (int r = 0; r < 16; ++r) {
                            const int row = 32 * rt + rho(r) + 4 * half;
                            const float val = rt < nt ? res[ti][r] : 0.f;
                            sdst[row * FS + hc + c] = val;
                        }
                    }
                }
            }
            lds_barrier();
        }
        {
            const long wofs = (long)KH * 64 + col;
            if (grp == 0) { load_wT<MM, 64, 64>(KARG(FusedBwdP, wq), wofs, wA); load_wT<MM, 32, 64>(KARG(FusedBwdP, wk), wofs, wk4); }
            else { load_wT<MM, 32, 64>(KARG(FusedBwdP, wk), wofs + 32 * 64, wk4); load_wT<MM, 64, 64>(KARG(FusedBwdP, wv), wofs, wA); }
            const float* const pX = KARG(FusedBwdP, X);
            e_bt = gld4(KARG(FusedBwdP, sqrt_beta) + lc);
#pragma unroll
            for (int i = 0; i < 2; ++i) e_x[i] = ald4<BF>(pX, (tok0 + min(32 * i + lr, L - 1)) * 64 + lc);
        }
#pragma unroll
        for (int i = 0; i < 2; ++i) {
            const int r = 32 * i + lr;
            if (r < L) {
                const long e = (tok0 + r) * 64 + lc;
                ast4<BF>(R6_dq, e, ld4(sQ + r * FS + lc));
                ast4<BF>(R6_dk, e, ld4(sK + r * FS + lc));
                ast4<BF>(R6_dv, e, ld4(sV + r * FS + lc));
            }
        }
    }

    STAMP(6);
    {
        f32x16 acc;
#pragma unroll
        for (int r = 0; r < 16; ++r) acc[r] = 0.f;
        mma_w<MM, 64>((grp == 0 ? sQ : sV) + arow, wA, acc);
        mma_w<MM, 32>(sK + arow + 32 * grp, wk4, acc);
        float* part = grp == 0 ? sG : sPm;
#pragma unroll
        for (int r = 0; r < 16; ++r) part[(wm * 32 + rho(r) + 4 * half) * FS + col] = acc[r];
    }
    lds_barrier();

    STAMP(7);
    const auto R8_dX = KARG(FusedBwdP, dX);
    const auto R8_pbeta = KARG(FusedBwdP, pbeta);
// ... 120 lines not shown
```

bsarec_amd/csrc/fused_top.h:

```cpp
#pragma once
#include "fused_layer.h"

struct TopFwdP {
    const float* X; float* Xout;
    const float *sqrt_beta, *f_g, *f_b, *wq, *bq, *wk, *bk, *wv, *bv, *wo, *bo, *a_g, *a_b, *w1, *b1, *w2, *b2, *ff_g, *ff_b;
    const float* tw; const int* ids32;
    float *xhat_f, *rstd_f, *q, *k, *v, *probs, *ctx, *xhat_a, *rstd_a, *hmix, *u, *xhat_ff, *rstd_ff;
    float* low;
    int L, Lp, cb, heads;
    float alpha, oma, eps;
    DropP drop_f, drop_p, drop_o, drop_ff;
    long long* stamps;
    const float *wk_sh, *wv_sh;
};

__device__ __forceinline__ float drop_mult1(const DropP& d, const DropSeed& sd, uint64_t e) {
    if (d.thresh == 0) return d.scale;
    const uint64_t grp = e >> 2;
    const uint4 w = philox4x32_10((uint32_t)grp, (uint32_t)(grp >> 32), d.site, sd.step, sd.k0, sd.k1);
    const int j = (int)(e & 3);
    const uint32_t r = j == 0 ? w.x : j == 1 ? w.y : j == 2 ? w.z : w.w;
    return r >= d.thresh ? d.scale : 0.f;
}

// ... 264 lines not shown
    lds_barrier();
    TSTAMP(6);

    if constexpr (!HELPED) {
        const float u = gemv_rows_dot<64, 1>(w1r, sHm, 0) + R.b1_n;
        ast<BF>(k_u, (tok0 + tl) * 256 + tid, u);
        sG[tid] = gelu_f(u);
    }
    lds_barrier();
    TSTAMP(7);
    if constexpr (!HELPED) {
        const float y = gemv_rows_dot<256, 4>(w2r, sG, osl) + R.b2_n;
        if (osl == 0) sQ[on] = y;
    }
    lds_barrier();
    TSTAMP(8);
    if (wave == 0) {
        const int c = lane;
        const float v = sQ[c] * (HELPED ? sMul[128 + c] : drop_mult1(d_ff, dseed, (uint64_t)(el + c))) + sHm[c];
        float xh, rs;
        ln_row(v, k_eps, xh, rs);
        ast<BF>(k_xhat_ff, el + c, xh);
        if (c == 0) gst(k_rstd_ff + tok0 + tl, rs);
        gst(k_Xout + el + c, R.c_ffg * xh + R.c_ffb);
    }
    TSTAMP(15);
}

template <bool BF>
struct TopFwdHelpRegs {
    WFrag<BF, 64> wA, wB;
    float bias_k, bias_v;
};
template <bool BF, unsigned KOFF>
__device__ __forceinline__ void top_fwd_help_prefetch(TopFwdHelpRegs<BF>& H) {
    const int lane = threadIdx.x & 63, hw = ((int)threadIdx.x >> 6) - 4;
    const int l31 = lane & 31, half = lane >> 5;
    const int wn = hw & 1, col = wn * 32 + l31;
    const int KH = (BF ? 8 : 4) * half;
    load_w<BF, 64>(BF ? TP(wv_sh) : TP(wv), (long)col * 64 + KH, H.wB);
    load_w<BF, 64>(BF ? TP(wk_sh) : TP(wk), (long)col * 64 + KH, H.wA);
    H.bias_v = gld(TP(bv) + col); H.bias_k = gld(TP(bk) + col);
}
template <int DH, bool BF, unsigned KOFF>
__device__ __forceinline__ void top_fwd_help(const TopFwdHelpRegs<BF>& H, const float* sX, float* sK, float* sV, float* sVec) {
    float* sQ = sVec; const float* sHm = sVec + 384; float* sG = sVec + 448;
    const int t = (int)threadIdx.x - 256, lane = t & 63, hw = t >> 6;
    const int l31 = lane & 31, half = lane >> 5;
    const int L = TP(L);
    const int b = blockIdx.x, tl = L - 1;
    const long tok0 = (long)b * L;
    const int wm = hw >> 1, wn = hw & 1, col = wn * 32 + l31;
    const int KH = (BF ? 8 : 4) * half;
    const float* const pW1 = TP(w1); const float* const pW2 = TP(w2);
    float* const Pk = TP(k); float* const Pv = TP(v); float* const k_u = TP(u);
    const int arow = (wm * 32 + l31) * FS + KH;
    {
        f32x16 acc;
#pragma unroll
        for (int r = 0; r < 16; ++r) acc[r] = 0.f;
        mma_w<BF, 64>(sX + arow, H.wB, acc);
#pragma unroll
        for (int r = 0; r < 16; ++r) sV[(wm * 32 + rho(r) + 4 * half) * FS + col] = acc[r] + H.bias_v;
    }
    lds_barrier();
    {
        f32x16 acc;
#pragma unroll
        for (int r = 0; r < 16; ++r) acc[r] = 0.f;
        mma_w<BF, 64>(sX + arow, H.wA, acc);
#pragma unroll
        for (int r = 0; r < 16; ++r) sK[(wm * 32 + rho(r) + 4 * half) * FS + col] = acc[r] + H.bias_k;
    }
    lds_barrier();
// ... 501 lines not shown
```

bsarec_amd/csrc/kernels.h:

```cpp
#pragma once
#include "common.h"

#define ROW_THREADS 256
#include "lazy_adam.h"

struct GatherP {
    const int64_t* table; const int64_t* ans_table; const int64_t* perm; long n;
    const long long* cursor; int64_t* ids_out; int64_t* ans_out;
};

template <int LPR>
__global__ void __launch_bounds__(ROW_THREADS)
embed_fwd_kernel(const int64_t* __restrict__ ids, GatherP gp, const float* __restrict__ E, const float* __restrict__ Pos,
                 const float* __restrict__ gamma, const float* __restrict__ beta, float eps, DropP drop,
                 int T, int L, int d, int V, float* __restrict__ X0, float* __restrict__ xhat,
                 float* __restrict__ rstd, int* __restrict__ ids32) {
    constexpr int RPB = ROW_THREADS / LPR;
    const int lr = threadIdx.x / LPR, lc = (threadIdx.x % LPR) << 2;
    const int tok = blockIdx.x * RPB + lr;
    const bool ok = tok < T && lc < d;
    f32x4 v = {0, 0, 0, 0};
    if (ok) {
        int64_t id64;
        if (gp.table) {
            const int b = tok / L, t = tok - b * L;
            long src = *gp.cursor + b;
            src = src < gp.n ? gp.perm[src] : 0;
            id64 = gp.table[src * L + t];
            if (lc == 0) {
                gp.ids_out[tok] = id64;
                if (t == 0) gp.ans_out[b] = gp.ans_table[src];
            }
        } else id64 = ids[tok];
        int id = (int)id64;
        id = id < 0 ? 0 : (id >= V ? V - 1 : id);
        if (lc == 0) ids32[tok] = id;
        v = ld4(E + (long)id * d + lc) + ld4(Pos + (long)(tok % L) * d + lc);
// ... 507 lines not shown
    constexpr int RPP = ROW_THREADS / LPR, W = LPR * 4;
    extern __shared__ __attribute__((aligned(16))) float esm[];
    const int lr = threadIdx.x / LPR, lc = (threadIdx.x % LPR) << 2;
    const bool colok = lc < d;
    if ((int)blockIdx.x < scatter_blocks) {
        embed_scatter_block<LPR>(de, ids32, B * L, d, dA, blockIdx.x, esm);
        return;
    }
    float (*red)[W] = reinterpret_cast<float (*)[W]>(esm);
    const int pb = blockIdx.x - scatter_blocks;
    const int t = pb % L, slice = pb / L;
    const int b0 = slice * 64, b1 = min(B, b0 + 64);
    f32x4 s0 = {0, 0, 0, 0}, s1 = s0, s2 = s0, s3 = s0;
    if (colok) {
        int bb = b0 + lr;
        for (; bb + 3 * RPP < b1; bb += 4 * RPP) {
            s0 += ld4(de + ((long)bb * L + t) * d + lc);
            s1 += ld4(de + ((long)(bb + RPP) * L + t) * d + lc);
            s2 += ld4(de + ((long)(bb + 2 * RPP) * L + t) * d + lc);
            s3 += ld4(de + ((long)(bb + 3 * RPP) * L + t) * d + lc);
        }
        for (; bb < b1; bb += RPP) s0 += ld4(de + ((long)bb * L + t) * d + lc);
    }
    st4(&red[lr][lc], (s0 + s1) + (s2 + s3));
    __syncthreads();
    for (int c = threadIdx.x; c < d; c += ROW_THREADS) {
        float a = 0.f;
#pragma unroll
        for (int g = 0; g < RPP; ++g) a += red[g][c];
        dPos[((long)slice * L + t) * d + c] = a;
    }
}

struct ReduceJob { const float* src; float* dst; int nsplit; int len; long stride; float scale; int pad; };

__device__ __forceinline__ void reduce_chunk(const ReduceJob& j, int chunk, float (*red)[64]) {
    const int e = threadIdx.x & 63, sg = threadIdx.x >> 6;
    const int i = chunk * 64 + e;
    float a[16];
#pragma unroll
    for (int k = 0; k < 16; ++k) a[k] = 0.f;
    if (i < j.len) {
        const float* p = j.src + i;
        int s = sg;
        for (; s + 60 < j.nsplit; s += 64) {
#pragma unroll
            for (int k = 0; k < 16; ++k) a[k] += p[(long)(s + 4 * k) * j.stride];
        }
        for (int k = 0; s < j.nsplit; s += 4, ++k) a[k & 15] += p[(long)s * j.stride];
    }
    float t = 0.f;
#pragma unroll
    for (int k = 0; k < 16; ++k) t += a[k];
    red[sg][e] = t;
    __syncthreads();
    if (sg == 0 && i < j.len) j.dst[i] = ((red[0][e] + red[1][e]) + (red[2][e] + red[3][e])) * j.scale;
}

struct ReduceJobs3 { ReduceJob j[3]; };
__global__ void __launch_bounds__(ROW_THREADS)
multi_reduce3_kernel(const ReduceJobs3 J) {
    __shared__ float red[4][64];
    const ReduceJob j = J.j[blockIdx.y];
    if (blockIdx.x * 64 >= j.len) return;
    reduce_chunk(j, blockIdx.x, red);
}

// ... 93 lines not shown
    for (long i = (long)blockIdx.x * ROW_THREADS + threadIdx.x; i < n4; i += (long)gridDim.x * ROW_THREADS) {
        f32x4 gi;
        if (S.nsrc > 0) {
            f32x4 part[8];
#pragma unroll
            for (int r = 0; r < 8; ++r) if (r < S.nsrc) part[r] = ld4_sys(S.src[r] + 4 * i);
            gi = part[0];
#pragma unroll
            for (int r = 1; r < 8; ++r) if (r < S.nsrc) gi += part[r];
        } else {
            gi = ld4(g + 4 * i);
            if (S.g2 && i < S.n2_4) { gi += ld4(S.g2 + 4 * i); st4(S.g2 + 4 * i, f32x4{0, 0, 0, 0}); }
        }
        gi = gi * gscale;
        f32x4 wi = ld4(w + 4 * i), mi = ld4(m + 4 * i), vi = ld4(v + 4 * i);
        if (wd != 0.f) gi += wd * wi;
        mi = b1 * mi + (1.0f - b1) * gi;
        vi = b2 * vi + (1.0f - b2) * gi * gi;
#pragma unroll
        for (int k = 0; k < 4; ++k) wi[k] -= step_size * (mi[k] / (sqrtf(vi[k]) / bc2s + eps));
        st4(w + 4 * i, wi); st4(m + 4 * i, mi); st4(v + 4 * i, vi);
        if (shadow && i >= shadow_from4)
            *reinterpret_cast<uint2*>(shadow + 4 * i) = make_uint2(adam_pk_bf16(wi.x, wi.y), adam_pk_bf16(wi.z, wi.w));
    }
}

struct AdamFuseP {
    float *w, *g, *m, *v; float b1, b2, eps, wd;
    unsigned short* shadow; long shadow_from;
    long item_off, item_n4;
    unsigned long long* lookup_acc;
    int dense_zero;
    LazyRows lazy;
};
__global__ void __launch_bounds__(ROW_THREADS)
reduce_adam_kernel(const ReduceJob* __restrict__ jobs, const int* __restrict__ blockmap, int nblocks,
                   const uint64_t* __restrict__ state, const AdamFuseP A) {
    __shared__ float red[ROW_THREADS];
    const float* f = reinterpret_cast<const float*>(state + 3);
    const float step_size = f[0], bc2s = f[1];
    if ((int)blockIdx.x < nblocks) {
        const int bm = blockmap[blockIdx.x];
        const ReduceJob j = jobs[bm >> 16];
        float (*r4)[64] = reinterpret_cast<float(*)[64]>(red);
        const int e = threadIdx.x & 63, sg = threadIdx.x >> 6, i = (bm & 0xFFFF) * 64 + e;
        float a[16];
#pragma unroll
        for (int k = 0; k < 16; ++k) a[k] = 0.f;
        if (i < j.len) {
            const float* p = j.src + i;
            int s = sg;
            for (; s + 60 < j.nsplit; s += 64) {
#pragma unroll
                for (int k = 0; k < 16; ++k) a[k] += p[(long)(s + 4 * k) * j.stride];
            }
            for (int k = 0; s < j.nsplit; s += 4, ++k) a[k & 15] += p[(long)s * j.stride];
        }
        float t = 0.f;
#pragma unroll
        for (int k = 0; k < 16; ++k) t += a[k];
        r4[sg][e] = t;
        __syncthreads();
        if (sg == 0 && i < j.len) {
            const float gi0 = ((r4[0][e] + r4[1][e]) + (r4[2][e] + r4[3][e])) * j.scale;
            j.dst[i] = gi0;
            const long o = (j.dst - A.g) + i;
            float wi = A.w[o], mi = A.m[o], vi = A.v[o], gi = gi0;
            if (A.wd != 0.f) gi += A.wd * wi;
            mi = A.b1 * mi + (1.0f - A.b1) * gi;
            vi = A.b2 * vi + (1.0f - A.b2) * gi * gi;
            wi -= step_size * (mi / (sqrtf(vi) / bc2s + A.eps));
            A.w[o] = wi; A.m[o] = mi; A.v[o] = vi;
            if (A.shadow && o >= A.shadow_from) A.shadow[o] = (unsigned short)(adam_pk_bf16(wi, 0.f) & 0xFFFFu);
        }
        return;
    }
    const long nb = gridDim.x - nblocks;
    if (A.lazy.rows) {
        lazy_adam_rows(A.lazy, (long)(blockIdx.x - nblocks) * ROW_THREADS + threadIdx.x, nb * ROW_THREADS, A.w, A.m, A.v, A.item_off,
                       A.b1, A.b2, A.eps, A.wd, step_size, bc2s, [&](long i, long o) {
                           f32x4 gi = {0, 0, 0, 0};
                           if (A.lookup_acc) lookup_take(A.lookup_acc, i, gi);
                           st4(A.g + o, gi);
                           return gi;
                       });
        return;
    }
    for (long i = (long)(blockIdx.x - nblocks) * ROW_THREADS + threadIdx.x; i < A.item_n4; i += nb * ROW_THREADS) {
        const long o = A.item_off + 4 * i;
        f32x4 wi = ld4(A.w + o), mi = ld4(A.m + o), vi = ld4(A.v + o);
        f32x4 gi = A.dense_zero ? f32x4{0, 0, 0, 0} : ld4(A.g + o);
        f32x4 add;
        if (A.lookup_acc && lookup_take(A.lookup_acc, i, add)) {
            gi = A.dense_zero ? add : gi + add;
            st4(A.g + o, gi);
        } else if (A.dense_zero) st4(A.g + o, gi);
        if (A.wd != 0.f) gi += A.wd * wi;
        mi = A.b1 * mi + (1.0f - A.b1) * gi;
        vi = A.b2 * vi + (1.0f - A.b2) * gi * gi;
#pragma unroll
        for (int k = 0; k < 4; ++k) wi[k] -= step_size * (mi[k] / (sqrtf(vi[k]) / bc2s + A.eps));
        st4(A.w + o, wi); st4(A.m + o, mi); st4(A.v + o, vi);
        if (A.shadow && o >= A.shadow_from)
            *reinterpret_cast<uint2*>(A.shadow + o) = make_uint2(adam_pk_bf16(wi.x, wi.y), adam_pk_bf16(wi.z, wi.w));
    }
}

struct CastJobs6 { const float* src[6]; unsigned short* dst[6]; long n4[6]; };
__global__ void __launch_bounds__(ROW_THREADS)
cast_bf16_kernel(const CastJobs6 J) {
    const float* src = J.src[blockIdx.y];
    unsigned short* dst = J.dst[blockIdx.y];
    const long i = (long)blockIdx.x * ROW_THREADS + threadIdx.x;
    if (i >= J.n4[blockIdx.y]) return;
    const f32x4 x = ld4(src + 4 * i);
    *reinterpret_cast<uint2*>(dst + 4 * i) = make_uint2(adam_pk_bf16(x.x, x.y), adam_pk_bf16(x.z, x.w));
}

__global__ void __launch_bounds__(ROW_THREADS)
loss_mean_kernel(const float* __restrict__ rows, int B, float* __restrict__ out) {
    __shared__ float red[ROW_THREADS];
    float s = 0.f;
    for (int i = threadIdx.x; i < B; i += ROW_THREADS) s += rows[i];
    red[threadIdx.x] = s;
    __syncthreads();
    for (int o = ROW_THREADS / 2; o > 0; o >>= 1) {
        if ((int)threadIdx.x < o) red[threadIdx.x] += red[threadIdx.x + o];
        __syncthreads();
    }
    if (threadIdx.x == 0) out[0] = red[0] / (float)B;
}

__global__ void __launch_bounds__(ROW_THREADS)
bce_rows_kernel(const float* __restrict__ hlast, long hstride, const float* __restrict__ E, const int64_t* __restrict__ pos,
                const int64_t* __restrict__ neg, int B, int d, int V, float* __restrict__ coef, float* __restrict__ loss_out,
                int logsig ) {
    __shared__ float red[2][ROW_THREADS];
    float lsum = 0.f, cnt = 0.f;
// ... 177 lines not shown
```

bsarec_amd/model.py:

```python
from __future__ import annotations

import ctypes as C
import math
from collections import OrderedDict
from typing import Dict, List, Optional, Tuple

import numpy as np
import torch
import torch.nn as nn

from . import _lib as L


def param_shapes(args) -> "OrderedDict[str, Tuple[int, ...]]":
    d, Lq, V = args.hidden_size, args.max_seq_length, args.item_size
    s: "OrderedDict[str, Tuple[int, ...]]" = OrderedDict()
    s["item_embeddings.weight"] = (V, d)
    s["position_embeddings.weight"] = (Lq, d)
    s["LayerNorm.weight"] = (d,)
    s["LayerNorm.bias"] = (d,)
    for l in range(args.num_hidden_layers):
        p = f"item_encoder.blocks.{l}."
        s[p + "layer.filter_layer.sqrt_beta"] = (1, 1, d)
        s[p + "layer.filter_layer.LayerNorm.weight"] = (d,)
# ... 27 lines not shown

class _Plan:

    def __init__(self, model: "BSARecModel", batch: int, garena=None, own_state: bool = False):
        lib = L.load()
        a = model.args
        self.cfg = L.Config(batch, a.max_seq_length, a.hidden_size, a.num_attention_heads, a.num_hidden_layers,
                            a.item_size, model.cutoff_bins, float(a.alpha), 1e-12, float(a.hidden_dropout_prob),
                            float(a.attention_probs_dropout_prob), int(getattr(a, "filter_kind", 0)))
        self.cfg.hidden_act = L.HIDDEN_ACTS[getattr(a, "hidden_act", "gelu")]
        opts = L.default_options()
        opts.update(model.options)
        for k in L.OPTION_FIELDS:
            setattr(self.cfg, k, int(opts.get(k, 0)))
        self.options = {k: int(getattr(self.cfg, k)) for k in L.OPTION_FIELDS}
        for k in L.TRAIN_FIELDS:
            setattr(self.cfg, k, model.train_head[k])
        self.cfg.train_lazy_adam = int(model.lazy_adam)
        nbytes = lib.bsarec_workspace_bytes(C.byref(self.cfg))
        if nbytes == 0:
            raise ValueError("configuration not supported by libbsarec_hip (see include/bsarec_hip.h limits: "
                             "L <= 256, hidden <= 256 and % 4 == 0, head size % 4 == 0, cutoff_bins*hidden <= 8192)")
        dev = model._arena.device
        self.ws = torch.empty(nbytes + 256, dtype=torch.uint8, device=dev)
        off = (-self.ws.data_ptr()) % 256
        self.ws = self.ws[off:off + nbytes]
        self.ws.zero_()
        self.batch = batch
        self.handle = C.c_void_p()
        self.bf16 = bool(self.cfg.storage) and lib.bsarec_config_is_fused(C.byref(self.cfg)) == 1
        self.garena = model._garena if garena is None else garena
        pt, gt = model._tensor_struct(model._arena), model._tensor_struct(self.garena)
        st = model._tensor_struct(model._shadow_arena()) if self.bf16 else None
        stream = torch.cuda.current_stream(dev).cuda_stream
        self.state = torch.zeros_like(model._state) if own_state else model._state
        L.check(lib.bsarec_plan_create(C.byref(self.handle), C.byref(self.cfg), C.byref(pt), C.byref(gt),
                                       C.byref(st) if st is not None else None,
                                       self.ws.data_ptr(), nbytes, self.state.data_ptr(),
                                       model._twiddle.data_ptr(), stream), "bsarec_plan_create")
        self.lib = lib
        if self.cfg.train_negatives > 0 and self.cfg.train_sampler == 1 and model._train_cum is not None:
            model._install_train_sampler(self)

    def view(self, buf: int, layer: int, shape) -> torch.Tensor:
        off = self.lib.bsarec_buffer_offset(self.handle, buf, layer)
        if off < 0:
            raise IndexError("no such buffer")
        if self.lib.bsarec_buffer_is_bf16(self.handle, buf, layer):
            n = int(np.prod(shape)) * 2
            return self.ws[off:off + n].view(torch.bfloat16).view(*shape)
        n = int(np.prod(shape)) * 4
        return self.ws[off:off + n].view(torch.float32).view(*shape)

    def __del__(self):
        try:
            if self.handle:
                self.lib.bsarec_plan_destroy(self.handle)
        except Exception:
            pass


class _SlotToken:

    def __init__(self, model, key):
        self.model, self.key = model, key

# ... 145 lines not shown
            for name in parts[:-1]:
                if not hasattr(mod, name):
                    mod.add_module(name, _Bag())
                mod = getattr(mod, name)
            mod.register_parameter(parts[-1], nn.Parameter(arena[o:o + n].view(shp)))

    def _grads_in_param_order(self, g):
        out = []
        for name, _ in self.named_parameters():
            o, n, shp = self._slices[name]
            out.append(g[o:o + n].view(shp))
        return tuple(out)

    def _param_by_key(self, key):
        mod = self
        parts = key.split(".")
        for name in parts[:-1]:
            mod = getattr(mod, name)
        return mod._parameters[parts[-1]]

    def _install_arena(self, arena):
        self._arena = arena
        self._garena = torch.zeros_like(arena)
        for key, (o, n, shp) in self._slices.items():
            p = self._param_by_key(key)
            p.data = arena[o:o + n].view(shp)
            p.grad = None
        self._state = torch.zeros(8, dtype=torch.int64, device=arena.device)
        self._twiddle = _twiddle(self.args.max_seq_length).to(arena.device)
        self._plans = {}
        self._adam = None
        self._shadow = None
        self._shadow_stale = True
        self._garena_alt = None
        self._lookup = None
        self._dense_hook = None

    def use_grad_arenas(self, arenas):
        assert all(a.numel() == self._numel and a.dtype == torch.float32 for a in arenas)
        self._garena, self._garena_alt = arenas[0], arenas[1]
        self._garena.zero_(); self._garena_alt.zero_()
        self._plans = {}

    def enable_lookup_grad(self):
        vd = self._slices["item_embeddings.weight"][1]
        self._gbuf = torch.zeros(self._numel + vd, dtype=torch.float32, device=self._arena.device)
        self._garena, self._lookup = self._gbuf[:self._numel], self._gbuf[self._numel:]
        self._plans = {}

    def set_dense_grad_hook(self, fn):
        self._dense_hook_py = fn
        self._dense_hook = L.HOOK(lambda user, stream: fn(stream)) if fn is not None else None
        for plan in self._plans.values():
            self._install_hook(plan)

    def set_train_popularity(self, counts):
        V = int(self.args.item_size)
        c = np.asarray(counts, dtype=np.int64)
        if c.shape != (V,) or (c < 0).any():
            raise ValueError(f"set_train_popularity: expected {V} counts >= 0")
        cum = np.cumsum(np.where(np.arange(V) == 0, 0, c))
        if cum[-1] < 1:
            raise ValueError("set_train_popularity: every count is 0")
        self._train_cum, self._train_cum_dev = cum, None
        for plan in self._plans.values():
            self._install_train_sampler(plan)

    def _install_train_sampler(self, plan):
        if plan.cfg.train_negatives == 0 or plan.cfg.train_sampler != 1:
            return
        dev = self._arena.device
        if self._train_cum_dev is None or self._train_cum_dev.device != dev:
            self._train_cum_dev = torch.as_tensor(self._train_cum, dtype=torch.int64, device=dev)
        L.check(plan.lib.bsarec_plan_set_train_sampler(plan.handle, self._train_cum_dev.data_ptr()),
                "bsarec_plan_set_train_sampler")
        plan._pop_keepalive = self._train_cum_dev

    def _install_hook(self, plan):
        lk = self._lookup.data_ptr() if (self._lookup is not None and plan.garena is self._garena) else None
        hook = self._dense_hook if self._dense_hook is not None else L.HOOK(0)
        L.check(plan.lib.bsarec_plan_set_dense_grad_hook(plan.handle, hook, None, lk), "bsarec_plan_set_dense_grad_hook")

    def _shadow_arena(self):
        if self._shadow is None:
            self._shadow = self._arena.to(torch.bfloat16)
            self._shadow_stale = True
        return self._shadow

    def _refresh_shadow(self, plan, force=False):
        if plan.bf16 and (force or self._shadow_stale):
            L.check(plan.lib.bsarec_shadow_refresh(plan.handle, self._stream()), "bsarec_shadow_refresh")
            self._shadow_stale = False

    def load_state_dict(self, state_dict, strict=True, **kw):
        out = super().load_state_dict(state_dict, strict=strict, **kw)
        self._shadow_stale = True
        return out

    def _apply(self, fn, recurse=True):
        out = super()._apply(fn, recurse)
        ref = self._param_by_key("item_embeddings.weight")
        arena = torch.empty(self._numel, dtype=torch.float32, device=ref.device)
        for key, (o, n, shp) in self._slices.items():
            arena[o:o + n] = self._param_by_key(key).data.reshape(-1).to(torch.float32)
        seed = self._seed if hasattr(self, "_seed") else 42
        self._install_arena(arena)
        self._seed = seed
        return out

    def init_weights(self, module=None):
        std = self.args.initializer_range
        with torch.no_grad():
            for key, (o, n, shp) in self._slices.items():
                p = self._param_by_key(key)
                if key.endswith("sqrt_beta"):
                    p.normal_(0.0, 1.0)
                elif key.endswith("complex_weight"):
                    p.normal_(0.0, 1.0).mul_(0.02)
                elif "LayerNorm.weight" in key:
                    p.fill_(1.0)
                elif key.endswith(".bias"):
                    p.zero_()
                else:
                    p.normal_(0.0, std)

    def _tensor_struct(self, arena) -> L.Tensors:
        t = L.Tensors()
        base, esz = arena.data_ptr(), arena.element_size()

# ... 26 lines not shown
        key = (batch, str(self._arena.device), tuple(sorted(opts.items())), parity, slot)
        if key not in self._plans:
            if int(self._state[0].item()) == 0:
                self.set_seed(self._seed)
            if slot > 0:
                self._plans[key] = _Plan(self, batch, own_state=True)
            elif parity == 0:
                self._plans[key] = _Plan(self, batch)
            else:
                self._plans[key] = _Plan(self, batch, garena=self._garena_alt)
            if self._lookup is not None or self._dense_hook is not None:
                self._install_hook(self._plans[key])
        return self._plans[key]

    def _stream(self):
        return torch.cuda.current_stream(self._arena.device).cuda_stream

    def _run_forward(self, input_ids, train: bool, new_step: bool, last_only: bool = False, slot: int = 0) -> _Plan:
        if input_ids.dim() != 2 or input_ids.shape[1] != self.args.max_seq_length:
            raise ValueError("input_ids must be [B, max_seq_length]")
        ids = input_ids.to(device=self._arena.device, dtype=torch.int64).contiguous()
        plan = self._plan(ids.shape[0], slot=slot)
        lib, st = plan.lib, self._stream()
        if new_step:
            if slot:
                self._state[1:2].add_(1)
            else:
                L.check(lib.bsarec_step_begin(plan.handle, st), "bsarec_step_begin")
            self._step_begun = True
        if slot:
            plan.state.copy_(self._state)
        self._refresh_shadow(plan, force=True)
        self._shadow_stale = True
        fwd = lib.bsarec_forward_last if last_only else lib.bsarec_forward
        L.check(fwd(plan.handle, ids.data_ptr(), 1 if train else 0, st), "bsarec_forward")
        plan._ids_keepalive = ids
        return plan

    def _fresh_step_counter(self, plan: _Plan):
        if getattr(self, "_step_begun", False):
            L.check(plan.lib.bsarec_step_begin(plan.handle, self._stream()), "bsarec_step_begin")
            self._step_begun = False

    def _run_loss(self, plan: _Plan, answers):
        ans = answers.to(device=self._arena.device, dtype=torch.int64).contiguous()
        L.check(plan.lib.bsarec_loss(plan.handle, ans.data_ptr(), self._stream()), "bsarec_loss")
        plan._ans_keepalive = ans

    def _run_backward(self, plan: _Plan):
        L.check(plan.lib.bsarec_backward(plan.handle, self._stream()), "bsarec_backward")

    def forward(self, input_ids, user_ids=None, all_sequence_output=False):
        B, Lq, d = input_ids.shape[0], self.args.max_seq_length, self.args.hidden_size
        if self.training and torch.is_grad_enabled() and any(p.requires_grad for p in self.parameters()):
            if all_sequence_output:
                return list(_SeqAllFn.apply(self, input_ids, *self.parameters()))
            return _SeqFn.apply(self, input_ids, *self.parameters())
        plan = self._run_forward(input_ids, train=self.training, new_step=self.training)
        if all_sequence_output:
            return [plan.view(L.BUF_LAYER_OUT, l, (B, Lq, d)).float().clone() for l in range(self.args.num_hidden_layers + 1)]
        return plan.view(L.BUF_LAYER_OUT, self.args.num_hidden_layers, (B, Lq, d)).clone()

    def predict(self, input_ids, user_ids=None, all_sequence_output=False):
        return self.forward(input_ids, user_ids, all_sequence_output)

    def calculate_loss(self, input_ids, answers, neg_answers=None, same_target=None, user_ids=None):
# ... 57 lines not shown
        if not hasattr(plan, "ids_buf"):
            dev = self._arena.device
            plan.ids_buf = torch.zeros((batch, self.args.max_seq_length), dtype=torch.int64, device=dev)
            plan.ans_buf = torch.zeros((batch,), dtype=torch.int64, device=dev)
        self._fresh_step_counter(plan)
        self._refresh_shadow(plan)
        ad = self._adam_struct()
        L.check(plan.lib.bsarec_train_step_indexed(
            plan.handle, table.data_ptr(), answers_table.data_ptr(), perm.data_ptr(), perm.shape[0], cursor.data_ptr(),
            plan.ids_buf.data_ptr(), plan.ans_buf.data_ptr(), C.byref(ad), self._stream()), "bsarec_train_step_indexed")
        return plan.view(L.BUF_LOSS, 0, (1,))[0]

    def grad_step_indexed(self, table, answers_table, perm, cursor, batch: int, tick_adam: bool = False,
                          parity: int = 0) -> torch.Tensor:
        plan = self._plan(batch, parity)
        if not hasattr(plan, "ids_buf"):
            dev = self._arena.device
            plan.ids_buf = torch.zeros((batch, self.args.max_seq_length), dtype=torch.int64, device=dev)
            plan.ans_buf = torch.zeros((batch,), dtype=torch.int64, device=dev)
        self._fresh_step_counter(plan)
        self._refresh_shadow(plan)
        L.check(plan.lib.bsarec_grad_step_indexed(
            plan.handle, table.data_ptr(), answers_table.data_ptr(), perm.data_ptr(), perm.shape[0], cursor.data_ptr(),
            plan.ids_buf.data_ptr(), plan.ans_buf.data_ptr(), self._adam["lr"] if tick_adam else 0.0,
            self._adam["b1"] if tick_adam else 0.0, self._adam["b2"] if tick_adam else 0.0, self._stream()),
            "bsarec_grad_step_indexed")
        return plan.view(L.BUF_LOSS, 0, (1,))[0]

    def adam_step(self, grad_scale: float = 1.0, tick: bool = True, grad_srcs=None):
        if self.lazy_adam:
            raise ValueError("adam_step: a lazy-Adam model updates inside train_step / train_step_indexed (a plan-less "
                             "update cannot know which item rows the step touched)")
        ad = self._adam_struct(grad_scale, grad_srcs)
        fn = L.load().bsarec_adam_step if tick else L.load().bsarec_adam_apply
        L.check(fn(C.byref(ad), self._state.data_ptr(), self._stream()), "bsarec_adam_step" if tick else "bsarec_adam_apply")

    def grad_views(self) -> "OrderedDict[str, torch.Tensor]":
        return OrderedDict((k, self._garena[o:o + n].view(shp)) for k, (o, n, shp) in self._slices.items())


class _BCEFn(torch.autograd.Function):

    @staticmethod
    def forward(ctx, model, ids, pos, neg, *params):
        plan = model._run_forward(ids, train=model.training, new_step=model.training, last_only=True)
        model._run_loss_bce(plan, pos, neg)
        ctx.model, ctx.plan = model, plan
        return plan.view(L.BUF_LOSS, 0, (1,))[0].clone()

    @staticmethod
    def backward(ctx, gout):
        model, plan = ctx.model, ctx.plan
        model._run_backward(plan)
        g = model._garena * gout
        return (None, None, None, None) + model._grads_in_param_order(g)


class SASRecModel(BSARecModel):

    needs_negatives = True
    sampled_softmax_ok = False

    def __init__(self, args):
        import copy
        a = copy.copy(args)
        a.alpha = 0.0
        if not hasattr(a, "c"):
            a.c = 3
# ... 203 lines not shown
```

bsarec_amd/trainer.py:

```python
from __future__ import annotations

import math
import os
from typing import Optional

import numpy as np
import torch

from .data import DeviceBatches
from .dp import PeerExchange, allreduce_sum_
from .model import BSARecModel


class _NullLogger:
    def info(self, *a, **k):
        pass


def recall_at_k(hit: torch.Tensor, k: int) -> float:
    return float(hit[:, :k].any(1).double().mean().item())


def ndcg_at_k(hit: torch.Tensor, k: int) -> float:
    w = 1.0 / torch.log2(torch.arange(k, device=hit.device, dtype=torch.float64) + 2.0)
# ... 120 lines not shown
        self._b1_done.record(self._side)

    def exchange_desc(self) -> str:
        if not self.dp:
            return "none (single GPU)"
        how = "one graph per step incl. the exchange" if (self.use_graph and self.dp_graph == "one") else \
            ("grad graph + eager exchange + Adam graph" if self.use_graph else "eager")
        what = {"rccl": "one RCCL all-reduce of the flat gradient arena after the backward",
                "rccl_bucketed": "two RCCL all-reduces: the dense item-table gradient on a side stream under the encoder backward, "
                                 "the encoder gradients + lookup rows after it",
                "p2p": "one cross-GPU barrier kernel, then the fused Adam reads every rank's IPC-mapped gradient arena over xGMI "
                       "(no collective library in the data path)"}[self.exchange]
        return f"{what}; {how}"

    def exchange_report(self) -> dict:
        m = self.model
        n = int(m._numel * 4)
        if self.exchange == "rccl_bucketed":
            vd = int(self._vd * 4)
            return {"kind": "rccl_bucketed", "buckets": 2, "overlapped_bytes": vd, "exposed_bytes": n, "launch": self.dp_graph}
        if self.exchange == "p2p":
            return {"kind": "p2p", "buckets": 0, "remote_read_bytes": n * (self.world - 1), "exposed": "1 barrier kernel + remote reads inside Adam",
                    "timed_out": self._px.timed_out(), "launch": self.dp_graph}
        return {"kind": "rccl", "buckets": 1, "exposed_bytes": n, "launch": self.dp_graph}

    def _sync_replicas(self):
        if self.pg is None or self.world == 1:
            return
        m = self.model
        seed = m._state[0].clone()
        for t in (m._arena, m._adam["m"], m._adam["v"], m._state):
            torch.distributed.broadcast(t, src=torch.distributed.get_global_rank(self.pg, 0), group=self.pg)
        m._state[0] = seed

    def train(self, epoch):
        return self.iteration(epoch, self.train_dataloader, train=True)

    def valid(self, epoch):
        self.args.train_matrix = self.args.valid_rating_matrix
        self._eval_tag = 1
        return self.iteration(epoch, self.eval_dataloader, train=False)

    def test(self, epoch):
        self.args.train_matrix = self.args.test_rating_matrix
        self._eval_tag = 2
        return self.iteration(epoch, self.test_dataloader, train=False)

    def check_exchange(self):
        if self._px is None:
            return
        bad = torch.tensor([1.0 if self._px.timed_out() else 0.0], device=self.device)
        if self.world > 1:
            torch.distributed.all_reduce(bad, op=torch.distributed.ReduceOp.MAX, group=self.pg)
        if bad.item() != 0.0:
            raise RuntimeError("peer-to-peer gradient exchange: a cross-GPU barrier timed out on some rank (the error word is "
                               "sticky); the replicas can no longer be trusted -- restart from the last checkpoint with "
                               "exchange='rccl'")

    def save(self, file_name):
        self.check_exchange()
        torch.save({k: v.detach().cpu() for k, v in self.model.state_dict().items()}, file_name)

    def load(self, file_name):
        sd = torch.load(file_name, map_location="cpu", weights_only=True)
        self.model.load_state_dict(sd)
        self._sync_replicas()
# ... 481 lines not shown
```

include/bsarec_hip.h:

```cpp
#ifndef BSAREC_HIP_H
#define BSAREC_HIP_H

#include <stddef.h>
#include <stdint.h>

#ifdef __cplusplus
extern "C" {
#endif

#define BSAREC_MAX_LAYERS 16
#define BSAREC_ABI_VERSION 10

typedef struct {
    int batch;
    int seq_len;
    int hidden;
    int heads;
    int layers;
    int item_size;
    int cutoff_bins;
    float alpha;
    float ln_eps;
    float p_hidden;
    float p_attn;
    int filter_kind;
    int hidden_act;
    int storage;
    int no_fused;
    int no_prune_top;
    int dw_tiled;
    int splits;
    int top_slabs;
    int separate_embed;
    int separate_top;
    int chain_kernels;
    int x3_products;
    int train_negatives;
    int train_sampler;
    int train_no_logq;
    int train_lazy_adam;
} bsarec_config_t;

typedef struct {
    float *sqrt_beta, *filter_ln_w, *filter_ln_b;
    float *query_w, *query_b, *key_w, *key_b, *value_w, *value_b, *dense_w, *dense_b;
    float *attn_ln_w, *attn_ln_b;
    float *ffn1_w, *ffn1_b, *ffn2_w, *ffn2_b, *ffn_ln_w, *ffn_ln_b;
    float *filter_cw;
} bsarec_layer_t;

typedef struct {
    float *item_emb;
    float *pos_emb;
    float *ln_w, *ln_b;
    bsarec_layer_t layer[BSAREC_MAX_LAYERS];
} bsarec_tensors_t;

enum {
    BSAREC_BUF_LAYER_OUT = 0,
    BSAREC_BUF_LOGITS = 1,
    BSAREC_BUF_LOSS = 2,
    BSAREC_BUF_DSP = 3,
    BSAREC_BUF_HMIX = 4,
    BSAREC_BUF_PROBS = 5,
    BSAREC_BUF_DLAYER_IN = 6,
    BSAREC_BUF_LOSS_ROWS = 7,
    BSAREC_BUF_CTX = 8,
    BSAREC_BUF_DLOGITS = 9,
    BSAREC_BUF_TRAIN_CAND = 10,
    BSAREC_BUF_TRAIN_CORR = 11,
    BSAREC_BUF_TRAIN_LOGITS = 12,
    BSAREC_BUF_TRAIN_DLOGITS = 13
};

typedef struct bsarec_plan bsarec_plan_t;

int bsarec_abi_version(void);

size_t bsarec_workspace_bytes(const bsarec_config_t *cfg);

#define BSAREC_STATE_BYTES 64

int bsarec_plan_create(bsarec_plan_t **out, const bsarec_config_t *cfg, const bsarec_tensors_t *params,
                       const bsarec_tensors_t *grads, const bsarec_tensors_t *shadow, void *workspace,
                       size_t workspace_bytes, void *state, const float *twiddle, void *stream);
int bsarec_shadow_refresh(bsarec_plan_t *plan, void *stream);
int bsarec_buffer_is_bf16(const bsarec_plan_t *plan, int buffer, int layer);

int bsarec_plan_is_fused(const bsarec_plan_t *plan);
int bsarec_config_is_fused(const bsarec_config_t *cfg);
void bsarec_plan_destroy(bsarec_plan_t *plan);

typedef void (*bsarec_hook_t)(void *user, void *stream);
int bsarec_plan_set_dense_grad_hook(bsarec_plan_t *plan, bsarec_hook_t hook, void *user, float *lookup_grad);

#define BSAREC_TRAIN_NEG_MAX 8192
#define BSAREC_TRAIN_NEG_SITE 0x4E454753u

int bsarec_plan_set_train_sampler(bsarec_plan_t *plan, const int64_t *pop_cum);

long bsarec_buffer_offset(const bsarec_plan_t *plan, int buffer, int layer);

int bsarec_step_begin(bsarec_plan_t *plan, void *stream);

int bsarec_forward(bsarec_plan_t *plan, const int64_t *ids, int train, void *stream);

int bsarec_loss(bsarec_plan_t *plan, const int64_t *answers, void *stream);

int bsarec_forward_last(bsarec_plan_t *plan, const int64_t *ids, int train, void *stream);

int bsarec_loss_bce(bsarec_plan_t *plan, const int64_t *pos_ids, const int64_t *neg_ids, void *stream);
int bsarec_loss_logsig(bsarec_plan_t *plan, const int64_t *pos_ids, const int64_t *neg_ids, void *stream);

int bsarec_logits(bsarec_plan_t *plan, void *stream);

int bsarec_backward(bsarec_plan_t *plan, void *stream);

int bsarec_backward_seq(bsarec_plan_t *plan, const float *d_out, void *stream);

int bsarec_backward_seq_multi(bsarec_plan_t *plan, const float *const *d_outs, void *stream);

typedef struct {
    float *params;
    const float *grads;
    float *exp_avg, *exp_avg_sq;
    long n;
    float lr, beta1, beta2, eps, weight_decay;
    float grad_scale;
    void *shadow_bf16;
    long shadow_from;
    float *grads2;
    long grads2_n;
    int n_grad_srcs;
    const float *grad_srcs[8];
} bsarec_adam_t;

int bsarec_adam_step(const bsarec_adam_t *adam, void *state, void *stream);
int bsarec_adam_apply(const bsarec_adam_t *adam, void *state, void *stream);

int bsarec_train_step(bsarec_plan_t *plan, const int64_t *ids, const int64_t *answers, const bsarec_adam_t *adam,
                      void *stream);

int bsarec_gather_batch(const int64_t *table, const int64_t *answers_table, const int64_t *perm, long n_samples,
                        const void *cursor, int B, int L, int64_t *ids_out, int64_t *answers_out, void *stream);

int bsarec_train_step_indexed(bsarec_plan_t *plan, const int64_t *table, const int64_t *answers_table,
                              const int64_t *perm, long n_samples, void *cursor, int64_t *ids_buf, int64_t *answers_buf,
                              const bsarec_adam_t *adam, void *stream);

int bsarec_grad_step_indexed(bsarec_plan_t *plan, const int64_t *table, const int64_t *answers_table,
                             const int64_t *perm, long n_samples, void *cursor, int64_t *ids_buf, int64_t *answers_buf,
                             float lr, float beta1, float beta2, void *stream);

int bsarec_mask_seen(float *scores, long ld, int B, const int64_t *users, const int64_t *indptr,
                     const int64_t *indices, void *stream);

#define BSAREC_TOPK_MAX 1024
int bsarec_topk_seen(float *scores, long ld, int B, int V, const int64_t *users, const int64_t *indptr,
                     const int64_t *indices, int k, int64_t *out_idx, float *out_val, void *stream);

#define BSAREC_NEG_MAX 1024
#define BSAREC_NEG_MAX_DRAWS (1 << 20)
int bsarec_sampled_rank(const float *h, long ldh, const float *item_emb, int B, int V, int d, const int64_t *users,
                        const int64_t *answers, const int64_t *indptr, const int64_t *indices, const int64_t *pop_cum,
                        int n_neg, uint64_t seed, uint32_t tag, int32_t *rank_out, int64_t *cand_out, float *score_out,
                        void *stream);

// ... 27 lines not shown
```

Baseline: 1.669 million.

## Keep fp32 weights in a pre-swizzled MFMA fragment image for fused layer kernels

Adds a per-layer weight image that stores each dense weight, plus its transpose, in the lane/fragment order the fp32 MFMA loads expect. The fused forward and backward kernels then read weights with contiguous per-lane vector loads instead of strided gathers. The image is kept current by writing it from the fused reduce+Adam kernel, or by a refresh kernel after a separate Adam step. This costs extra memory and extra scattered stores during the optimizer update, and it risks stale weights if some update path misses a refresh.

```diff
diff --git a/bsarec_amd/_lib.py b/bsarec_amd/_lib.py
--- a/bsarec_amd/_lib.py
+++ b/bsarec_amd/_lib.py
@@ -43,17 +43,20 @@
                 ("dw_tiled", C.c_int), ("splits", C.c_int), ("top_slabs", C.c_int), ("separate_embed", C.c_int),
                 ("separate_top", C.c_int), ("chain_kernels", C.c_int), ("x3_products", C.c_int),
                 ("train_negatives", C.c_int), ("train_sampler", C.c_int), ("train_no_logq", C.c_int),
-                ("train_lazy_adam", C.c_int)]
+                ("train_lazy_adam", C.c_int),
+                ("weight_image", C.c_int)]
 
 
 TRAIN_FIELDS = ("train_negatives", "train_sampler", "train_no_logq")
 TRAIN_SAMPLERS = {"uniform": 0, "popularity": 1}
 
 
-OPTION_FIELDS = ("storage", "no_fused", "no_prune_top", "dw_tiled", "splits", "top_slabs", "separate_embed", "separate_top", "chain_kernels", "x3_products")
+OPTION_FIELDS = ("storage", "no_fused", "no_prune_top", "dw_tiled", "splits", "top_slabs", "separate_embed", "separate_top", "chain_kernels", "x3_products",
+                 "weight_image")
 HIDDEN_ACTS = {"gelu": 0, "relu": 1, "swish": 2, "tanh": 3, "sigmoid": 4}
 
 _defaults = {k: 0 for k in OPTION_FIELDS}
+_defaults["weight_image"] = 1
 
 
 def _env_defaults():
@@ -78,6 +81,8 @@
             d[key] = int(e[env])
     if e.get("BSAREC_STORAGE") == "bf16":
         d["storage"] = 1
+    if e.get("BSAREC_WEIGHT_IMAGE") == "0":
+        d["weight_image"] = 0
     return d
 
 
@@ -110,7 +115,8 @@
     _fields_ = [("params", C.c_void_p), ("grads", C.c_void_p), ("exp_avg", C.c_void_p), ("exp_avg_sq", C.c_void_p),
                 ("n", C.c_long), ("lr", C.c_float), ("beta1", C.c_float), ("beta2", C.c_float), ("eps", C.c_float),
                 ("weight_decay", C.c_float), ("grad_scale", C.c_float), ("shadow_bf16", C.c_void_p), ("shadow_from", C.c_long),
-                ("grads2", C.c_void_p), ("grads2_n", C.c_long), ("n_grad_srcs", C.c_int), ("grad_srcs", C.c_void_p * 8)]
+                ("grads2", C.c_void_p), ("grads2_n", C.c_long), ("n_grad_srcs", C.c_int), ("grad_srcs", C.c_void_p * 8),
+                ("wimage_plan", C.c_void_p)]
 
 
 class Comm(C.Structure):
@@ -127,6 +133,9 @@
     "bsarec_plan_create": (C.c_int, [C.POINTER(C.c_void_p), C.POINTER(Config), C.POINTER(Tensors), C.POINTER(Tensors),
                                      C.POINTER(Tensors), C.c_void_p, C.c_size_t, C.c_void_p, C.c_void_p, C.c_void_p]),
     "bsarec_shadow_refresh": (C.c_int, [C.c_void_p, C.c_void_p]),
+    "bsarec_wimage_refresh": (C.c_int, [C.c_void_p, C.c_void_p]),
+    "bsarec_wimage_floats": (C.c_long, [C.POINTER(Config)]),
+    "bsarec_wimage_offset": (C.c_long, [C.c_int] * 5),
     "bsarec_plan_set_dense_grad_hook": (C.c_int, [C.c_void_p, HOOK, C.c_void_p, C.c_void_p]),
     "bsarec_plan_set_train_sampler": (C.c_int, [C.c_void_p, C.c_void_p]),
     "bsarec_buffer_is_bf16": (C.c_int, [C.c_void_p, C.c_int, C.c_int]),
diff --git a/bsarec_amd/csrc/bsarec_hip.hip b/bsarec_amd/csrc/bsarec_hip.hip
--- a/bsarec_amd/csrc/bsarec_hip.hip
+++ b/bsarec_amd/csrc/bsarec_hip.hip
@@ -92,6 +92,7 @@
     int ssm_nslab = 0;
     LazyRows lazy = {};
     bool lazy_now = false;
+    float* wimg = nullptr;
 };
 struct PlanScope {
     bsarec_plan* prev;
@@ -199,7 +200,13 @@
     if (c.train_sampler < 0 || c.train_sampler > 1 || c.train_no_logq < 0 || c.train_no_logq > 1) return -17;
     if (c.train_negatives > 0 && c.storage != 0) return -18;
     if (c.train_lazy_adam < 0 || c.train_lazy_adam > 1 || (c.train_lazy_adam && c.train_negatives == 0)) return -19;
-    return 0;
+    if (c.weight_image < 0 || c.weight_image > 1) return -20;
+    return 0;
+}
+
+static bool fused_shape_ok(const bsarec_config_t& c);
+static bool wimage_wanted(const bsarec_config_t& c) {
+    return c.weight_image && fused_shape_ok(c) && c.storage == 0 && !c.x3_products && !c.chain_kernels && c.filter_kind == 0;
 }
 
 static bool fused_shape_ok(const bsarec_config_t& c) {
@@ -335,12 +342,26 @@
 static const float* h_last(const bsarec_plan& p) { return p.X[p.cfg.layers] + (long)(p.cfg.seq_len - 1) * p.cfg.hidden; }
 static long h_last_stride(const bsarec_plan& p) { return (long)p.cfg.seq_len * p.cfg.hidden; }
 
+static float* wimage_weight(const bsarec_plan& p, int l, int which, bool transposed) {
+    const long d = p.cfg.hidden;
+    return p.wimg + l * wimage_layer_floats(d) + (transposed ? 12 * d * d : 0) + wimage_weight_off(which, d);
+}
+static bsarec_layer_t wimage_layer(const bsarec_plan& p, int l, bool transposed) {
+    bsarec_layer_t w;
+    memset(&w, 0, sizeof(w));
+    w.query_w = wimage_weight(p, l, WIMAGE_WQ, transposed); w.key_w = wimage_weight(p, l, WIMAGE_WK, transposed);
+    w.value_w = wimage_weight(p, l, WIMAGE_WV, transposed); w.dense_w = wimage_weight(p, l, WIMAGE_WO, transposed);
+    w.ffn1_w = wimage_weight(p, l, WIMAGE_W1, transposed); w.ffn2_w = wimage_weight(p, l, WIMAGE_W2, transposed);
+    return w;
+}
+
 extern "C" int bsarec_plan_create(bsarec_plan_t** out, const bsarec_config_t* cfg, const bsarec_tensors_t* params,
                                   const bsarec_tensors_t* grads, const bsarec_tensors_t* shadow, void* workspace,
                                   size_t workspace_bytes, void* state, const float* twiddle, void* stream) {
     if (!out || !cfg || !params || !workspace || !state || !twiddle) return -10;
     RET(check_cfg(*cfg));
     if (cfg->storage == 1 && fused_shape_ok(*cfg) && !shadow) return -15;
+    if (wimage_wanted(*cfg) && (!shadow || !shadow->layer[0].query_w || ((uintptr_t)shadow->layer[0].query_w & 255))) return -15;
     if (((uintptr_t)workspace & 255) != 0) return -11;
     bsarec_plan* p = new bsarec_plan();
     p->cfg = *cfg;
@@ -349,6 +370,7 @@
     if (shadow) p->S = *shadow; else memset(&p->S, 0, sizeof(p->S));
     p->ws = (char*)workspace; p->ws_bytes = workspace_bytes;
     p->state = (uint64_t*)state; p->twiddle = twiddle; p->train = false;
+    p->wimg = wimage_wanted(*cfg) ? shadow->layer[0].query_w : nullptr;
     derive(*p);
     size_t total = 0;
     carve(*p, p->ws, &total);
@@ -369,19 +391,26 @@
         jobs.push_back(j);
     };
     const int ns = p->nsplit, nb = p->nblk;
+    auto add_w = [&](int l, int which, const float* src, float* dst) {
+        add(src, dst, ns, (which >= WIMAGE_W1 ? 4 : 1) * d * d);
+        if (!p->wimg) return;
+        ReduceJob& j = jobs.back();
+        j.img_f = wimage_weight(*p, l, which, false); j.img_t = wimage_weight(*p, l, which, true);
+        j.wn = (int)(which == WIMAGE_W1 ? 4 * d : d); j.wk = (int)(which == WIMAGE_W2 ? 4 * d : d);
+    };
     for (int l = 0; l < cfg->layers; ++l) {
         const bsarec_layer_t& g = p->G.layer[l];
         add(p->part_betaL[l], g.sqrt_beta, cfg->batch, d);
         add(ln_part(*p, l, LN_F_G), g.filter_ln_w, nb, d);
         add(ln_part(*p, l, LN_F_B), g.filter_ln_b, nb, d);
-        add(slab_w_ptr(*p, l, sm.wq), g.query_w, ns, d * d); add(slab_b_ptr(*p, l, sm.bq), g.query_b, ns, d);
-        add(slab_w_ptr(*p, l, sm.wk), g.key_w, ns, d * d);   add(slab_b_ptr(*p, l, sm.bk), g.key_b, ns, d);
-        add(slab_w_ptr(*p, l, sm.wv), g.value_w, ns, d * d); add(slab_b_ptr(*p, l, sm.bv), g.value_b, ns, d);
-        add(slab_w_ptr(*p, l, sm.wo), g.dense_w, ns, d * d); add(slab_b_ptr(*p, l, sm.bo), g.dense_b, ns, d);
+        add_w(l, WIMAGE_WQ, slab_w_ptr(*p, l, sm.wq), g.query_w); add(slab_b_ptr(*p, l, sm.bq), g.query_b, ns, d);
+        add_w(l, WIMAGE_WK, slab_w_ptr(*p, l, sm.wk), g.key_w);   add(slab_b_ptr(*p, l, sm.bk), g.key_b, ns, d);
+        add_w(l, WIMAGE_WV, slab_w_ptr(*p, l, sm.wv), g.value_w); add(slab_b_ptr(*p, l, sm.bv), g.value_b, ns, d);
+        add_w(l, WIMAGE_WO, slab_w_ptr(*p, l, sm.wo), g.dense_w); add(slab_b_ptr(*p, l, sm.bo), g.dense_b, ns, d);
         add(ln_part(*p, l, LN_A_G), g.attn_ln_w, nb, d);
         add(ln_part(*p, l, LN_A_B), g.attn_ln_b, nb, d);
-        add(slab_w_ptr(*p, l, sm.w1), g.ffn1_w, ns, 4 * d * d); add(slab_b_ptr(*p, l, sm.b1), g.ffn1_b, ns, 4 * d);
-        add(slab_w_ptr(*p, l, sm.w2), g.ffn2_w, ns, 4 * d * d); add(slab_b_ptr(*p, l, sm.b2), g.ffn2_b, ns, d);
+        add_w(l, WIMAGE_W1, slab_w_ptr(*p, l, sm.w1), g.ffn1_w); add(slab_b_ptr(*p, l, sm.b1), g.ffn1_b, ns, 4 * d);
+        add_w(l, WIMAGE_W2, slab_w_ptr(*p, l, sm.w2), g.ffn2_w); add(slab_b_ptr(*p, l, sm.b2), g.ffn2_b, ns, d);
         add(ln_part(*p, l, LN_FF_G), g.ffn_ln_w, nb, d);
         add(ln_part(*p, l, LN_FF_B), g.ffn_ln_b, nb, d);
     }
@@ -506,6 +535,33 @@
         case BSAREC_BUF_DLAYER_IN: return 1;
         default: return 0;
     }
+}
+
+extern "C" int bsarec_wimage_refresh(bsarec_plan_t* p, void* stream) {
+    if (!p) return -10;
+    if (!p->wimg) return 0;
+    WImageP W;
+    memset(&W, 0, sizeof(W));
+    for (int l = 0; l < p->cfg.layers; ++l) {
+        const bsarec_layer_t& w = p->P.layer[l];
+        const float* src[WIMAGE_NW] = {w.query_w, w.key_w, w.value_w, w.dense_w, w.ffn1_w, w.ffn2_w};
+        for (int i = 0; i < WIMAGE_NW; ++i) W.w[l][i] = src[i];
+    }
+    W.img = p->wimg; W.d = p->cfg.hidden;
+    LAUNCH(wimage_refresh_kernel, dim3(cdiv(12L * W.d * W.d, ROW_THREADS), p->cfg.layers), dim3(ROW_THREADS), 0, (hipStream_t)stream, W);
+    return g_dry ? 0 : (int)hipGetLastError();
+}
+
+extern "C" long bsarec_wimage_floats(const bsarec_config_t* cfg) {
+    if (!cfg || check_cfg(*cfg) != 0) return -10;
+    return wimage_wanted(*cfg) ? cfg->layers * wimage_layer_floats(cfg->hidden) : 0;
+}
+
+extern "C" long bsarec_wimage_offset(int which, int transposed, int d, int n, int k) {
+    if (which < 0 || which >= WIMAGE_NW || d < 32 || d % 32 || transposed < 0 || transposed > 1) return -1;
+    const int wn = which == WIMAGE_W1 ? 4 * d : d, wk = which == WIMAGE_W2 ? 4 * d : d;
+    if (n < 0 || n >= wn || k < 0 || k >= wk) return -1;
+    return (transposed ? 12L * d * d : 0) + wimage_weight_off(which, d) + (transposed ? wimage_off(k, n, wn) : wimage_off(n, k, wk));
 }
 
 extern "C" int bsarec_shadow_refresh(bsarec_plan_t* p, void* stream) {
@@ -635,7 +691,7 @@
                             bool top_tail = false ) {
     const bsarec_config_t& c = p.cfg;
     FusedFwdP F;
-    fill_block<true>(p, l, tr, p.bf ? p.S.layer[l] : p.P.layer[l], F);
+    fill_block<true>(p, l, tr, p.bf ? p.S.layer[l] : p.wimg ? wimage_layer(p, l, false) : p.P.layer[l], F);
     F.xout_f32 = (l == c.layers - 1);
     F.gp = p.lb[l].gp;
     F.dsp = nullptr;
@@ -646,7 +702,10 @@
     }
     F.trash = p.trash;
     TopFwdP TF;
-    if (top_tail) fill_top_fwd(p, l + 1, tr, TF);
+    if (top_tail) {
+        fill_top_fwd(p, l + 1, tr, TF);
+        if (p.wimg) { TF.wk_sh = wimage_weight(p, l + 1, WIMAGE_WK, false); TF.wv_sh = wimage_weight(p, l + 1, WIMAGE_WV, false); }
+    }
     const dim3 grid(c.batch), block(512);
     ProfScope prof(BSAREC_K_FUSED_FWD, s);
     if (c.filter_kind == 1) {
@@ -661,6 +720,11 @@
         return rc;
     }
     const size_t smem = fused_fwd_smem_bytes();
+    if (p.wimg) {
+        DISPATCH_DH(p.dh, rc = top_tail ? launch_lds<fused_layer_fwd_kernel<DH, false, TopFwdP, false, false, true>>(grid, block, smem, s, F, TF)
+                                        : launch_lds<fused_layer_fwd_kernel<DH, false, NoTail, false, false, true>>(grid, block, smem, s, F, NoTail()));
+        return rc;
+    }
     DISPATCH_BLOCK(p, rc = top_tail ? launch_lds<fused_layer_fwd_kernel<DH, BF, TopFwdP, X3>>(grid, block, smem, s, F, TF)
                                     : launch_lds<fused_layer_fwd_kernel<DH, BF, NoTail, X3>>(grid, block, smem, s, F, NoTail()));
     return rc;
@@ -670,7 +734,7 @@
                             const TopBwdP* head = nullptr ) {
     const bsarec_config_t& c = p.cfg;
     FusedBwdP F;
-    fill_block<false>(p, l, tr, p.bf ? p.S.layer[l] : p.P.layer[l], F);
+    fill_block<false>(p, l, tr, p.bf ? p.S.layer[l] : p.wimg ? wimage_layer(p, l, true) : p.P.layer[l], F);
     fill_block_partials(p, l, F);
     F.dY = dY; F.dX = dXout;
     F.u = p.lb[l].gp;
@@ -690,6 +754,11 @@
         return launch_lds<fused_layer_bwd_kernel<32, false, NoTail, false, true>>(grid, block, smem, s, F, NoTail());
     }
     int rc = 0;
+    if (p.wimg) {
+        DISPATCH_DH(p.dh, rc = head ? launch_lds<fused_layer_bwd_kernel<DH, false, TopBwdP, false, false, true>>(grid, block, smem, s, F, *head)
+                                    : launch_lds<fused_layer_bwd_kernel<DH, false, NoTail, false, false, true>>(grid, block, smem, s, F, NoTail()));
+        return rc;
+    }
     DISPATCH_BLOCK(p, rc = head ? launch_lds<fused_layer_bwd_kernel<DH, BF, TopBwdP, X3>>(grid, block, smem, s, F, *head)
                                 : launch_lds<fused_layer_bwd_kernel<DH, BF, NoTail, X3>>(grid, block, smem, s, F, NoTail()));
     return rc;
@@ -1290,6 +1359,13 @@
     return 0;
 }
 
+static bool adam_on_masters(const bsarec_plan& p, const bsarec_adam_t& a) {
+    return p.G.item_emb && a.params + (p.G.item_emb - a.grads) == p.P.item_emb;
+}
+static int wimage_after_adam(bsarec_plan& p, const bsarec_adam_t& a, hipStream_t s) {
+    return (p.wimg && !a.wimage_plan && adam_on_masters(p, a)) ? bsarec_wimage_refresh(&p, s) : 0;
+}
+
 static int final_reduce(bsarec_plan& p, const TickP& tick, const bsarec_adam_t* fuse_adam, hipStream_t s) {
     const bsarec_config_t& c = p.cfg;
     LookupAcc la;
@@ -1312,6 +1388,7 @@
         A.shadow = (unsigned short*)a.shadow_bf16; A.shadow_from = a.shadow_bf16 ? a.shadow_from : a.n;
         A.item_off = p.G.item_emb - a.grads; A.item_n4 = la.n4; A.lookup_acc = la.acc;
         A.dense_zero = la.dense_zero;
+        A.wimage = (p.wimg && adam_on_masters(p, a)) ? 1 : 0;
         if (lazy) A.lazy = p.lazy;
         int ab = lazy ? la.nblocks : cdiv(A.item_n4, ROW_THREADS);
         if (ab > 1024) ab = 1024;
@@ -1403,7 +1480,8 @@
     LAUNCH(adam_kernel, dim3(blocks), dim3(ROW_THREADS), 0, s, a.params, a.grads, a.exp_avg, a.exp_avg_sq, n4,
            (const uint64_t*)state, a.beta1, a.beta2, a.eps, a.weight_decay, a.grad_scale, (unsigned short*)a.shadow_bf16,
            a.shadow_bf16 ? a.shadow_from / 4 : n4, S);
-    return (int)hipGetLastError();
+    HIPCHK(hipGetLastError());
+    return a.wimage_plan ? bsarec_wimage_refresh(a.wimage_plan, s) : 0;
 }
 
 extern "C" int bsarec_adam_step(const bsarec_adam_t* a, void* state, void* stream) {
@@ -1475,7 +1553,8 @@
     if (can_fuse_adam(*p, *a) && !p->cfg.separate_embed)
         return backward_impl(p, stream, tk, a);
     RET(backward_impl(p, stream, tk));
-    return p->lazy_now ? lazy_adam_launch(*p, *a, s) : adam_launch(*a, p->state, s);
+    RET(p->lazy_now ? lazy_adam_launch(*p, *a, s) : adam_launch(*a, p->state, s));
+    return wimage_after_adam(*p, *a, s);
 }
 
 extern "C" int bsarec_grad_step_indexed(bsarec_plan_t* p, const int64_t* table, const int64_t* answers_table,
@@ -1503,13 +1582,15 @@
         RET(bsarec_loss(p, answers, stream));
         TickP tk = make_tick(p->state, 1, a->lr, a->beta1, a->beta2, nullptr, 0, nullptr, nullptr, 0, 0);
         RET(backward_impl(p, stream, tk));
-        return lazy_adam_launch(*p, *a, (hipStream_t)stream);
+        RET(lazy_adam_launch(*p, *a, (hipStream_t)stream));
+        return wimage_after_adam(*p, *a, (hipStream_t)stream);
     }
     RET(bsarec_step_begin(p, stream));
     RET(bsarec_forward_last(p, ids, 1, stream));
     RET(bsarec_loss(p, answers, stream));
     RET(bsarec_backward(p, stream));
-    return bsarec_adam_step(a, p->state, stream);
+    RET(bsarec_adam_step(a, p->state, stream));
+    return wimage_after_adam(*p, *a, (hipStream_t)stream);
 }
 
 extern "C" int bsarec_mask_seen(float* scores, long ld, int B, const int64_t* users, const int64_t* indptr,
diff --git a/bsarec_amd/csrc/fused_layer.h b/bsarec_amd/csrc/fused_layer.h
--- a/bsarec_amd/csrc/fused_layer.h
+++ b/bsarec_amd/csrc/fused_layer.h
@@ -1,6 +1,7 @@
 #pragma once
 #include "common.h"
 #include "kernels.h"
+#include "wimage.h"
 #include <type_traits>
 
 #define FS 68
@@ -188,9 +189,14 @@
     return mfma_bf16(a.h, b.h, acc);
 }
 
-template <int MM, int K>
+template <int MM, int K, int KT = 64, bool IMG = false>
 __device__ __forceinline__ void load_w(const float* __restrict__ base, long e, WFrag<MM, K>& f) {
-    if constexpr (MM == 1) {
+    static_assert(!IMG || MM == 0, "the fragment image exists for the fp32 products only");
+    if constexpr (IMG) {
+        const float* gw = base + wimage_off((int)(e / KT), (int)(e % KT), KT);
+#pragma unroll
+        for (int kb = 0; kb < K / 8; ++kb) f.w[kb] = gld4(gw + 256 * kb);
+    } else if constexpr (MM == 1) {
 #pragma unroll
         for (int s = 0; s < K / 16; ++s) f.w[s] = *reinterpret_cast<const AS_GLOBAL u32x4*>((const AS_GLOBAL char*)base + 2 * (e + 16 * s));
     } else if constexpr (MM == 2) {
@@ -201,9 +207,14 @@
         for (int kb = 0; kb < K / 8; ++kb) f.w[kb] = gld4(base + e + 8 * kb);
     }
 }
-template <int MM, int K, int LDW>
+template <int MM, int K, int LDW, int NR = 64, bool IMG = false>
 __device__ __forceinline__ void load_wT(const float* __restrict__ base, long e, WFrag<MM, K>& f) {
-    if constexpr (MM == 1) {
+    static_assert(!IMG || MM == 0, "the fragment image exists for the fp32 products only");
+    if constexpr (IMG) {
+        const float* gw = base + wimage_off((int)(e % LDW), (int)(e / LDW), NR);
+#pragma unroll
+        for (int kb = 0; kb < K / 8; ++kb) f.w[kb] = gld4(gw + 256 * kb);
+    } else if constexpr (MM == 1) {
         const AS_GLOBAL unsigned short* g = reinterpret_cast<const AS_GLOBAL unsigned short*>((const AS_GLOBAL char*)base + 2 * e);
 #pragma unroll
         for (int s = 0; s < K / 16; ++s) {
@@ -320,7 +331,7 @@
 __device__ __forceinline__ void top_fwd_rest(const TopFwdRegs<BF>& R, const DropSeed& dseed, float* sX, float* sK, float* sV,
                                              float* sPart, float* sTab, float* sSpec, float* sVec, const int* sIds);
 template <bool BF> struct TopFwdHelpRegs;
-template <bool BF, unsigned KOFF> __device__ __forceinline__ void top_fwd_help_prefetch(TopFwdHelpRegs<BF>& H);
+template <bool BF, unsigned KOFF, bool IMG> __device__ __forceinline__ void top_fwd_help_prefetch(TopFwdHelpRegs<BF>& H);
 template <int DH, bool BF, unsigned KOFF>
 __device__ __forceinline__ void top_fwd_help(const TopFwdHelpRegs<BF>& H, const float* sX, float* sK, float* sV, float* sVec);
 template <class T> struct IsTail { static constexpr bool value = true; };
@@ -343,11 +354,12 @@
 template <int DH, bool BF, unsigned KOFF> __device__ __forceinline__ void top_bwd_help_b(const float* sX, float* sVec, const float* gu, f32x4 (&uw)[16]);
 
 
-template <int DH, bool BF, class TAILP, bool X3 = false, bool FM = false>
+template <int DH, bool BF, class TAILP, bool X3 = false, bool FM = false, bool IMG = false>
 __global__ void __launch_bounds__(512) __attribute__((amdgpu_waves_per_eu(2, 2)))
 fused_layer_fwd_kernel(const FusedFwdP P_unused, const TAILP T_unused) {
 #define PTYPE FusedFwdP
     static_assert(!(BF && X3), "x3 products work on fp32 tensors");
+    static_assert(!IMG || (!BF && !X3 && !FM), "the fragment image feeds the fp32 products of the BSARec block");
     constexpr int MM = X3 ? 2 : (BF ? 1 : 0);
     static_assert(!FM || (!BF && !X3 && !IsTail<TAILP>::value), "the FMLPRec block runs in fp32, without a top-block tail");
     constexpr int MAXCB = FM ? 36 : FUSED_MAX_CB;
@@ -399,7 +411,7 @@
     WFrag<MM, 64> wA, wB;
     float qkv_bias[3] = {0.f, 0.f, 0.f};
     if (!FM && grp == 1) {
-        load_w<MM, 64>(R1_wq, wrow, wA);
+        load_w<MM, 64, 64, IMG>(R1_wq, wrow, wA);
         qkv_bias[0] = gld(KARG(FusedFwdP, bq) + col); qkv_bias[1] = gld(KARG(FusedFwdP, bk) + col);
         qkv_bias[2] = gld(KARG(FusedFwdP, bv) + col);
     }
@@ -492,8 +504,8 @@
             f32x16 acc;
 #pragma unroll
             for (int r = 0; r < 16; ++r) acc[r] = 0.f;
-            if (which == 0) { load_w<MM, 64>(R2_wk, wrow, wB); mma_w<MM, 64>(sX + arow, wA, acc); }
-            else if (which == 1) { load_w<MM, 64>(R2_wv, wrow, wA); mma_w<MM, 64>(sX + arow, wB, acc); }
+            if (which == 0) { load_w<MM, 64, 64, IMG>(R2_wk, wrow, wB); mma_w<MM, 64>(sX + arow, wA, acc); }
+            else if (which == 1) { load_w<MM, 64, 64, IMG>(R2_wv, wrow, wA); mma_w<MM, 64>(sX + arow, wB, acc); }
             else mma_w<MM, 64>(sX + arow, wA, acc);
             const float bias = qkv_bias[which];
 #pragma unroll
@@ -594,7 +606,7 @@
         }
     }
     WFrag<MM, 32> wO;
-    if constexpr (!FM) load_w<MM, 32>(R2_wo, wrow + 32 * grp, wO);
+    if constexpr (!FM) load_w<MM, 32, 64, IMG>(R2_wo, wrow + 32 * grp, wO);
     lds_barrier();
     if constexpr (!FM) {
     {
@@ -748,7 +760,7 @@
     LnPre lnA;
     if constexpr (!FM) lnA = ln_pre(R4_bo, R4_a_g, R4_a_b, R4_drop_o, dseed, tok0);
     {
-        load_w<MM, 64>(R4_w1, (long)(128 * grp + col) * 64 + KH, wA);
+        load_w<MM, 64, 64, IMG>(R4_w1, (long)(128 * grp + col) * 64 + KH, wA);
         ffn_bias[0] = gld(KARG(FusedFwdP, b1) + 128 * grp + col); ffn_bias[1] = gld(KARG(FusedFwdP, b1) + 128 * grp + 64 + col);
         if constexpr (!FM) {
         f32x16 acc;
@@ -778,8 +790,8 @@
             const int c256 = (2 * grp + i) * 64 + col;
             WFrag<MM, 64>& wcur = i ? wB : wA;
             WFrag<MM, 64>& wnxt = i ? wA : wB;
-            if (i == 0) load_w<MM, 64>(R5_w1, (long)(c256 + 64) * 64 + KH, wnxt);
-            else load_w<MM, 64>(R5_w2, (long)col * 256 + 128 * grp + KH, wnxt);
+            if (i == 0) load_w<MM, 64, 64, IMG>(R5_w1, (long)(c256 + 64) * 64 + KH, wnxt);
+            else load_w<MM, 64, 256, IMG>(R5_w2, (long)col * 256 + 128 * grp + KH, wnxt);
             f32x16 acc;
 #pragma unroll
             for (int r = 0; r < 16; ++r) acc[r] = 0.f;
@@ -819,7 +831,7 @@
 #pragma unroll
         for (int r = 0; r < 16; ++r) acc[r] = 0.f;
         const float* sa = sU + (wm * 32 + l31) * FU + 128 * grp + KH;
-        load_w<MM, 64>(R6_w2, (long)col * 256 + 128 * grp + 64 + KH, wB);
+        load_w<MM, 64, 256, IMG>(R6_w2, (long)col * 256 + 128 * grp + 64 + KH, wB);
         mma_w<MM, 64>(sa, wA, acc);
         mma_w<MM, 64>(sa + 64, wB, acc);
         float* part = grp == 0 ? sX : sE;
@@ -830,7 +842,7 @@
     STAMP(7);
     TopFwdRegs<BF> TR;
     TopFwdHelpRegs<BF> TH;
-    if constexpr (TAIL) { if (wave < 4) top_fwd_prefetch<BF, KOFF, false>(TR); else top_fwd_help_prefetch<BF, KOFF>(TH); }
+    if constexpr (TAIL) { if (wave < 4) top_fwd_prefetch<BF, KOFF, false>(TR); else top_fwd_help_prefetch<BF, KOFF, IMG>(TH); }
     const auto R7_Xout = KARG(FusedFwdP, Xout);
     const auto R7_eps = KARG(FusedFwdP, eps);
     const auto R7_rstd_ff = KARG(FusedFwdP, rstd_ff);
@@ -910,11 +922,12 @@
     }
 }
 
-template <int DH, bool BF, class HEADP, bool X3 = false, bool FM = false>
+template <int DH, bool BF, class HEADP, bool X3 = false, bool FM = false, bool IMG = false>
 __global__ void __launch_bounds__(512) __attribute__((amdgpu_waves_per_eu(2, 2)))
 fused_layer_bwd_kernel(const FusedBwdP P_unused, const HEADP H_unused) {
 #define PTYPE FusedBwdP
     static_assert(!(BF && X3), "x3 products work on fp32 tensors");
+    static_assert(!IMG || (!BF && !X3 && !FM), "the fragment image feeds the fp32 products of the BSARec block");
     constexpr int MM = X3 ? 2 : (BF ? 1 : 0);
     static_assert(!FM || (!BF && !X3 && !IsTail<HEADP>::value), "the FMLPRec block runs in fp32, without a top-block head");
     constexpr bool HEAD = IsTail<HEADP>::value;
@@ -994,7 +1007,7 @@
     WFrag<MM, 64> wA, wB;
     WFrag<MM, 32> wk4;
     f32x4 e_bt, e_x[2];
-    load_wT<MM, 64, 256>(R1_w2, (long)KH * 256 + 128 * grp + col, wA);
+    load_wT<MM, 64, 256, 64, IMG>(R1_w2, (long)KH * 256 + 128 * grp + col, wA);
     const f32x4 g = gld4(R1_ff_g + lc);
     f32x4 dy[2], xh[2];
     float rs[2];
@@ -1072,12 +1085,12 @@
     if constexpr (MM == 0) {
         const float* sa = sT + arow;
         const int c0 = (2 * grp) * 64 + col, c1 = c0 + 64;
-        load_wT<MM, 64, 256>(R2_w2, (long)KH * 256 + c1, wB);
+        load_wT<MM, 64, 256, 64, IMG>(R2_w2, (long)KH * 256 + c1, wB);
         f32x16 acc0, acc1;
 #pragma unroll
         for (int r = 0; r < 16; ++r) { acc0[r] = 0.f; acc1[r] = 0.f; }
         mma_w<MM, 64>(sa, wA, acc0);
-        load_wT<MM, 64, 64>(R2_w1, (long)(128 * grp + KH) * 64 + col, wA);
+        load_wT<MM, 64, 64, 256, IMG>(R2_w1, (long)(128 * grp + KH) * 64 + col, wA);
 #pragma unroll
         for (int r = 0; r < 16; ++r) {
             const f32x4 a = ld4(sa + 8 * (r >> 1));
@@ -1101,8 +1114,8 @@
             const int blk = 2 * grp + i, c256 = blk * 64 + col;
             WFrag<MM, 64>& wcur = i ? wB : wA;
             WFrag<MM, 64>& wnxt = i ? wA : wB;
-            if (i == 0) load_wT<MM, 64, 256>(R2_w2, (long)KH * 256 + c256 + 64, wnxt);
-            else load_wT<MM, 64, 64>(R2_w1, (long)(128 * grp + KH) * 64 + col, wnxt);
+            if (i == 0) load_wT<MM, 64, 256, 64, IMG>(R2_w2, (long)KH * 256 + c256 + 64, wnxt);
+            else load_wT<MM, 64, 64, 256, IMG>(R2_w1, (long)(128 * grp + KH) * 64 + col, wnxt);
             f32x16 acc;
 #pragma unroll
             for (int r = 0; r < 16; ++r) acc[r] = 0.f;
@@ -1132,8 +1145,8 @@
 #pragma unroll
         for (int r = 0; r < 16; ++r) acc[r] = 0.f;
         const float* sa = sdU + (wm * 32 + l31) * FU + 128 * grp + KH;
-        load_wT<MM, 64, 64>(R3_w1, (long)(128 * grp + 64 + KH) * 64 + col, wB);
-        if constexpr (!FM) load_wT<MM, 32, 64>(R3_wo, (long)(32 * grp + KH) * 64 + col, wO);
+        load_wT<MM, 64, 64, 256, IMG>(R3_w1, (long)(128 * grp + 64 + KH) * 64 + col, wB);
+        if constexpr (!FM) load_wT<MM, 32, 64, 64, IMG>(R3_wo, (long)(32 * grp + KH) * 64 + col, wO);
 #pragma unroll
         for (int i = 0; i < 2; ++i) {
             const int r = 32 * i + lr;
@@ -1513,8 +1526,8 @@
         }
         {
             const long wofs = (long)KH * 64 + col;
-            if (grp == 0) { load_wT<MM, 64, 64>(KARG(FusedBwdP, wq), wofs, wA); load_wT<MM, 32, 64>(KARG(FusedBwdP, wk), wofs, wk4); }
-            else { load_wT<MM, 32, 64>(KARG(FusedBwdP, wk), wofs + 32 * 64, wk4); load_wT<MM, 64, 64>(KARG(FusedBwdP, wv), wofs, wA); }
+            if (grp == 0) { load_wT<MM, 64, 64, 64, IMG>(KARG(FusedBwdP, wq), wofs, wA); load_wT<MM, 32, 64, 64, IMG>(KARG(FusedBwdP, wk), wofs, wk4); }
+            else { load_wT<MM, 32, 64, 64, IMG>(KARG(FusedBwdP, wk), wofs + 32 * 64, wk4); load_wT<MM, 64, 64, 64, IMG>(KARG(FusedBwdP, wv), wofs, wA); }
             const float* const pX = KARG(FusedBwdP, X);
             e_bt = gld4(KARG(FusedBwdP, sqrt_beta) + lc);
 #pragma unroll
diff --git a/bsarec_amd/csrc/fused_top.h b/bsarec_amd/csrc/fused_top.h
--- a/bsarec_amd/csrc/fused_top.h
+++ b/bsarec_amd/csrc/fused_top.h
@@ -320,14 +320,14 @@
     WFrag<BF, 64> wA, wB;
     float bias_k, bias_v;
 };
-template <bool BF, unsigned KOFF>
+template <bool BF, unsigned KOFF, bool IMG>
 __device__ __forceinline__ void top_fwd_help_prefetch(TopFwdHelpRegs<BF>& H) {
     const int lane = threadIdx.x & 63, hw = ((int)threadIdx.x >> 6) - 4;
     const int l31 = lane & 31, half = lane >> 5;
     const int wn = hw & 1, col = wn * 32 + l31;
     const int KH = (BF ? 8 : 4) * half;
-    load_w<BF, 64>(BF ? TP(wv_sh) : TP(wv), (long)col * 64 + KH, H.wB);
-    load_w<BF, 64>(BF ? TP(wk_sh) : TP(wk), (long)col * 64 + KH, H.wA);
+    load_w<BF, 64, 64, IMG>(BF || IMG ? TP(wv_sh) : TP(wv), (long)col * 64 + KH, H.wB);
+    load_w<BF, 64, 64, IMG>(BF || IMG ? TP(wk_sh) : TP(wk), (long)col * 64 + KH, H.wA);
     H.bias_v = gld(TP(bv) + col); H.bias_k = gld(TP(bk) + col);
 }
 template <int DH, bool BF, unsigned KOFF>
diff --git a/bsarec_amd/csrc/kernels.h b/bsarec_amd/csrc/kernels.h
--- a/bsarec_amd/csrc/kernels.h
+++ b/bsarec_amd/csrc/kernels.h
@@ -3,6 +3,7 @@
 
 #define ROW_THREADS 256
 #include "lazy_adam.h"
+#include "wimage.h"
 
 struct GatherP {
     const int64_t* table; const int64_t* ans_table; const int64_t* perm; long n;
@@ -576,7 +577,10 @@
     }
 }
 
-struct ReduceJob { const float* src; float* dst; int nsplit; int len; long stride; float scale; int pad; };
+struct ReduceJob {
+    const float* src; float* dst; int nsplit; int len; long stride; float scale; int pad;
+    float* img_f = nullptr; float* img_t = nullptr; int wn = 0, wk = 0;
+};
 
 __device__ __forceinline__ void reduce_chunk(const ReduceJob& j, int chunk, float (*red)[64]) {
     const int e = threadIdx.x & 63, sg = threadIdx.x >> 6;
@@ -736,6 +740,7 @@
     unsigned long long* lookup_acc;
     int dense_zero;
     LazyRows lazy;
+    int wimage;
 };
 __global__ void __launch_bounds__(ROW_THREADS)
 reduce_adam_kernel(const ReduceJob* __restrict__ jobs, const int* __restrict__ blockmap, int nblocks,
@@ -776,6 +781,7 @@
             wi -= step_size * (mi / (sqrtf(vi) / bc2s + A.eps));
             A.w[o] = wi; A.m[o] = mi; A.v[o] = vi;
             if (A.shadow && o >= A.shadow_from) A.shadow[o] = (unsigned short)(adam_pk_bf16(wi, 0.f) & 0xFFFFu);
+            if (A.wimage && j.img_f) wimage_store(j.img_f, j.img_t, i / j.wk, i % j.wk, j.wn, j.wk, wi);
         }
         return;
     }
@@ -808,6 +814,19 @@
         if (A.shadow && o >= A.shadow_from)
             *reinterpret_cast<uint2*>(A.shadow + o) = make_uint2(adam_pk_bf16(wi.x, wi.y), adam_pk_bf16(wi.z, wi.w));
     }
+}
+
+struct WImageP { const float* w[BSAREC_MAX_LAYERS][WIMAGE_NW]; float* img; int d; };
+__global__ void __launch_bounds__(ROW_THREADS)
+wimage_refresh_kernel(const WImageP P) {
+    const long d = P.d, dd = d * d;
+    const long i = (long)blockIdx.x * ROW_THREADS + threadIdx.x;
+    if (i >= 12 * dd) return;
+    const int which = i < 4 * dd ? (int)(i / dd) : (i < 8 * dd ? WIMAGE_W1 : WIMAGE_W2);
+    const int e = (int)(i - wimage_weight_off(which, d));
+    const int wn = which == WIMAGE_W1 ? 4 * P.d : P.d, wk = which == WIMAGE_W2 ? 4 * P.d : P.d;
+    float* f = P.img + blockIdx.y * wimage_layer_floats(d) + wimage_weight_off(which, d);
+    wimage_store(f, f + 12 * dd, e / wk, e % wk, wn, wk, P.w[blockIdx.y][which][e]);
 }
 
 struct CastJobs6 { const float* src[6]; unsigned short* dst[6]; long n4[6]; };
diff --git a/bsarec_amd/csrc/wimage.h b/bsarec_amd/csrc/wimage.h
--- /dev/null
+++ b/bsarec_amd/csrc/wimage.h
@@ -0,0 +1,18 @@
+#pragma once
+#include <hip/hip_runtime.h>
+
+__host__ __device__ inline long wimage_off(int col, int k, int kdim) {
+    const int tile = col >> 5, kb = k >> 3, lane = (col & 31) + 32 * ((k >> 2) & 1);
+    return ((long)(tile * (kdim >> 3) + kb) * 64 + lane) * 4 + (k & 3);
+}
+
+enum { WIMAGE_WQ, WIMAGE_WK, WIMAGE_WV, WIMAGE_WO, WIMAGE_W1, WIMAGE_W2, WIMAGE_NW };
+__host__ __device__ inline long wimage_weight_off(int which, long d) { return (which < 4 ? which : 4 * which - 12) * d * d; }
+__host__ __device__ inline long wimage_layer_floats(long d) { return 2 * 12 * d * d; }
+
+#ifdef __HIPCC__
+__device__ __forceinline__ void wimage_store(float* __restrict__ f, float* __restrict__ t, int n, int k, int wn, int wk, float v) {
+    f[wimage_off(n, k, wk)] = v;
+    t[wimage_off(k, n, wn)] = v;
+}
+#endif
diff --git a/bsarec_amd/model.py b/bsarec_amd/model.py
--- a/bsarec_amd/model.py
+++ b/bsarec_amd/model.py
@@ -83,6 +83,10 @@
         self.garena = model._garena if garena is None else garena
         pt, gt = model._tensor_struct(model._arena), model._tensor_struct(self.garena)
         st = model._tensor_struct(model._shadow_arena()) if self.bf16 else None
+        self.wimage = lib.bsarec_wimage_floats(C.byref(self.cfg)) > 0
+        if self.wimage:
+            st = L.Tensors()
+            st.layer[0].query_w = model._wimage_arena(lib.bsarec_wimage_floats(C.byref(self.cfg))).data_ptr()
         stream = torch.cuda.current_stream(dev).cuda_stream
         self.state = torch.zeros_like(model._state) if own_state else model._state
         L.check(lib.bsarec_plan_create(C.byref(self.handle), C.byref(self.cfg), C.byref(pt), C.byref(gt),
@@ -294,6 +298,8 @@
         self._adam = None
         self._shadow = None
         self._shadow_stale = True
+        self._wimage = None
+        self._wimage_stale = True
         self._garena_alt = None
         self._lookup = None
         self._dense_hook = None
@@ -349,14 +355,30 @@
             self._shadow_stale = True
         return self._shadow
 
+    def _wimage_arena(self, floats: int):
+        if self._wimage is None:
+            buf = torch.zeros(floats + 64, dtype=torch.float32, device=self._arena.device)
+            off = ((-buf.data_ptr()) % 256) // 4
+            self._wimage = buf[off:off + floats]
+            self._wimage_stale = True
+        assert self._wimage.numel() == floats
+        return self._wimage
+
     def _refresh_shadow(self, plan, force=False):
         if plan.bf16 and (force or self._shadow_stale):
             L.check(plan.lib.bsarec_shadow_refresh(plan.handle, self._stream()), "bsarec_shadow_refresh")
             self._shadow_stale = False
+        if plan.wimage and (force or self._wimage_stale):
+            L.check(plan.lib.bsarec_wimage_refresh(plan.handle, self._stream()), "bsarec_wimage_refresh")
+            self._wimage_stale = False
+
+    def weights_changed(self):
+        self._shadow_stale = True
+        self._wimage_stale = True
 
     def load_state_dict(self, state_dict, strict=True, **kw):
         out = super().load_state_dict(state_dict, strict=strict, **kw)
-        self._shadow_stale = True
+        self.weights_changed()
         return out
 
     def _apply(self, fn, recurse=True):
@@ -449,6 +471,7 @@
             plan.state.copy_(self._state)
         self._refresh_shadow(plan, force=True)
         self._shadow_stale = True
+        self._wimage_stale = True
         fwd = lib.bsarec_forward_last if last_only else lib.bsarec_forward
         L.check(fwd(plan.handle, ids.data_ptr(), 1 if train else 0, st), "bsarec_forward")
         plan._ids_keepalive = ids
@@ -572,8 +595,14 @@
             raise ValueError("adam_step: a lazy-Adam model updates inside train_step / train_step_indexed (a plan-less "
                              "update cannot know which item rows the step touched)")
         ad = self._adam_struct(grad_scale, grad_srcs)
+        plan = next((p for p in self._plans.values() if p.wimage), None)
+        if plan is not None:
+            ad.wimage_plan = plan.handle
+        elif self._wimage is not None:
+            self._wimage_stale = True
         fn = L.load().bsarec_adam_step if tick else L.load().bsarec_adam_apply
         L.check(fn(C.byref(ad), self._state.data_ptr(), self._stream()), "bsarec_adam_step" if tick else "bsarec_adam_apply")
+
 
     def grad_views(self) -> "OrderedDict[str, torch.Tensor]":
         return OrderedDict((k, self._garena[o:o + n].view(shp)) for k, (o, n, shp) in self._slices.items())
diff --git a/bsarec_amd/trainer.py b/bsarec_amd/trainer.py
--- a/bsarec_amd/trainer.py
+++ b/bsarec_amd/trainer.py
@@ -176,6 +176,7 @@
         for t in (m._arena, m._adam["m"], m._adam["v"], m._state):
             torch.distributed.broadcast(t, src=torch.distributed.get_global_rank(self.pg, 0), group=self.pg)
         m._state[0] = seed
+        m.weights_changed()
 
     def train(self, epoch):
         return self.iteration(epoch, self.train_dataloader, train=True)
diff --git a/include/bsarec_hip.h b/include/bsarec_hip.h
--- a/include/bsarec_hip.h
+++ b/include/bsarec_hip.h
@@ -39,6 +39,7 @@
     int train_sampler;
     int train_no_logq;
     int train_lazy_adam;
+    int weight_image;
 } bsarec_config_t;
 
 typedef struct {
@@ -85,6 +86,9 @@
                        const bsarec_tensors_t *grads, const bsarec_tensors_t *shadow, void *workspace,
                        size_t workspace_bytes, void *state, const float *twiddle, void *stream);
 int bsarec_shadow_refresh(bsarec_plan_t *plan, void *stream);
+int bsarec_wimage_refresh(bsarec_plan_t *plan, void *stream);
+long bsarec_wimage_floats(const bsarec_config_t *cfg);
+long bsarec_wimage_offset(int which, int transposed, int d, int n, int k);
 int bsarec_buffer_is_bf16(const bsarec_plan_t *plan, int buffer, int layer);
 
 int bsarec_plan_is_fused(const bsarec_plan_t *plan);
@@ -133,6 +137,7 @@
     long grads2_n;
     int n_grad_srcs;
     const float *grad_srcs[8];
+    bsarec_plan_t *wimage_plan;
 } bsarec_adam_t;
 
 int bsarec_adam_step(const bsarec_adam_t *adam, void *state, void *stream);
```

After: 1.719 million, median of 6. 3.0% higher.
